# Daniel-Liu-c0deb0t/block-aligner

Hardware: AMD Instinct MI355X
Metric: GCUPS (DP cells/s) on 10 kbp DNA X-drop batch; bit-exact score+CIGAR vs AVX2 (higher is better)
Workload: dtype i16 (saturating lane scores) + i32 block offsets

## Files before the change

block_aligner_amd/csrc/ba_host.cpp:

```cpp
#include <hip/hip_runtime.h>

#include <algorithm>
#include <functional>
#include <cmath>
#include <cstdarg>
#include <cstdio>
#include <cstdlib>
#include <cstring>
#include <map>
#include <memory>
#include <string>
#include <type_traits>
#include <vector>
#include <atomic>
#include <chrono>
#include <thread>

#include "../../include/block_aligner_hip.h"
#include "aa_matrices.inc"
#include "ba_launch.h"

using ba::BatchParams;
using ba::BlockRec;

typedef const ba::KernelEntry* KernelTable[2][ba::N_KINDS][ba::N_CLASSES][ba::FAM_COUNT];
static KernelTable& kernel_table() { static KernelTable t = {}; return t; }
int ba::register_kernels(int kind, int pmax, bool special, const ba::KernelEntry* entries, int n) {
    int pc = 0;
    while ((1 << pc) < pmax) pc++;
    for (int k = 0; k < n; k++) kernel_table()[special][kind][pc][entries[k].family] = &entries[k];
    return n;
}
static const ba::KernelEntry* find_kernel(int family, int kind, int pc, int special) {
    if (family < 0 || family >= ba::FAM_COUNT || kind < 0 || kind >= ba::N_KINDS || pc < 0 || pc >= ba::N_CLASSES || special < 0 || special > 1) return nullptr;
    return kernel_table()[special][kind][pc][family];
}
constexpr int BA_PCLASS_BIG = 5;
static inline int special_of(uint32_t mode) { return (mode & (BA_LOCAL_START | BA_FREE_QUERY_START_GAPS | BA_FREE_QUERY_END_GAPS)) ? 1 : 0; }
constexpr int BA_KIND_PROFILE_ = ba::KIND_PROFILE;

#ifdef BA_DEV
#define dev_env(name) getenv(name)
#else
#define dev_env(name) ((const char*)nullptr)
#endif
#ifndef BA_BUILD_ID
#define BA_BUILD_ID "unknown"
#endif
extern "C" const char* ba_build_id(void) { return BA_BUILD_ID; }
extern "C" int ba_dev_build(void) {
#ifdef BA_DEV
    return 1;
#else
    return 0;
#endif
}

static thread_local std::string g_err;
static int fail(const char* fmt, ...) {
    char buf[512];
    va_list ap; va_start(ap, fmt); vsnprintf(buf, sizeof buf, fmt, ap); va_end(ap);
    g_err = buf;
    return 1;
}
[[noreturn]] static void die(const char* fmt, ...) {
    char buf[512];
    va_list ap; va_start(ap, fmt); vsnprintf(buf, sizeof buf, fmt, ap); va_end(ap);
    fprintf(stderr, "block_aligner_hip: %s\n", buf);
    abort();
}
#define HIP_TRY(expr) do { hipError_t e_ = (expr); if (e_ != hipSuccess) return fail("%s failed: %s", #expr, hipGetErrorString(e_)); } while (0)

static thread_local int g_device = -1;
static int ensure_device() {
    int n = 0;
    hipError_t e = hipGetDeviceCount(&n);
    if (e != hipSuccess || n <= 0) return fail("no usable HIP device (hipGetDeviceCount: %s); block_aligner_hip has no CPU fallback", hipGetErrorString(e));
    if (g_device < 0) g_device = 0;
    HIP_TRY(hipSetDevice(g_device));
    return 0;
}

struct AAMatrix { alignas(32) int8_t scores[27 * 32]; };
struct NucMatrix { alignas(32) int8_t scores[8 * 16]; };

static constexpr AAMatrix expand_tri(const signed char* tri) {
    AAMatrix m{};
    for (int k = 0; k < 27 * 32; k++) m.scores[k] = -128;
    int idx = 0;
    const char* letters = BA_AA_LETTERS;
    for (int a = 0; a < BA_AA_NLETTERS; a++)
        for (int b = 0; b <= a; b++) {
            const int ia = letters[a] - 'A', ib = letters[b] - 'A';
            m.scores[ia * 32 + ib] = tri[idx];
            m.scores[ib * 32 + ia] = tri[idx];
            idx++;
        }
    return m;
}
static constexpr NucMatrix nuc_simple(int8_t match, int8_t mismatch) {
    NucMatrix m{};
    for (int k = 0; k < 8 * 16; k++) m.scores[k] = -128;
    const char alpha[5] = {'A', 'T', 'C', 'G', 'N'};
    for (int i = 0; i < 5; i++)
        for (int j = 0; j < 5; j++) m.scores[(alpha[i] & 7) * 16 + (alpha[j] & 15)] = i == j ? match : mismatch;
    return m;
}
extern "C" {
extern const NucMatrix NW1 = nuc_simple(1, -1);
extern const AAMatrix BLOSUM45 = expand_tri(BA_TRI_BLOSUM45);
extern const AAMatrix BLOSUM50 = expand_tri(BA_TRI_BLOSUM50);
extern const AAMatrix BLOSUM62 = expand_tri(BA_TRI_BLOSUM62);
extern const AAMatrix BLOSUM80 = expand_tri(BA_TRI_BLOSUM80);
extern const AAMatrix BLOSUM90 = expand_tri(BA_TRI_BLOSUM90);
extern const AAMatrix PAM100 = expand_tri(BA_TRI_PAM100);
extern const AAMatrix PAM120 = expand_tri(BA_TRI_PAM120);
extern const AAMatrix PAM160 = expand_tri(BA_TRI_PAM160);
extern const AAMatrix PAM200 = expand_tri(BA_TRI_PAM200);
extern const AAMatrix PAM250 = expand_tri(BA_TRI_PAM250);
extern const ByteMatrix BYTES1 = {1, -1};
}

static inline uint8_t upper(uint8_t c) { return (c >= 'a' && c <= 'z') ? (uint8_t)(c - 32) : c; }
static inline int seq_kind(int kind) { return kind == BA_KIND_PROFILE_ ? BA_KIND_AA : kind; }
static inline uint8_t null_byte(int kind) { kind = seq_kind(kind); return kind == BA_KIND_AA ? 26 : (kind == BA_KIND_NUC ? 'Z' : 0); }
static inline bool convert_char(int kind, uint8_t c, uint8_t* out) {
    kind = seq_kind(kind);
    if (kind == BA_KIND_BYTES) { *out = c; return true; }
    c = upper(c);
    if (kind == BA_KIND_AA) { if (c < 'A' || c > 'A' + 26) return false; *out = (uint8_t)(c - 'A'); return true; }
    if (c < 'A' || c > 'Z') return false;
    *out = c;
    return true;
}

struct PaddedBytes {
    std::vector<uint8_t> s;
    size_t len;
    int kind;
};
struct Cigar {
    std::vector<OpLen> ops;
    size_t capacity;
};
struct AAProfile {
    std::vector<int8_t> pos_aa;
    std::vector<int16_t> gap_open_C, gap_close_C, gap_open_R;
    int8_t gap_extend;
    size_t max_len, curr_len, str_len;
};

struct DevBuf {
    void* p = nullptr;
    size_t bytes = 0;
    bool owned = true;
    void view(void* q, size_t n) { free_(); p = q; bytes = n; owned = false; }
    int alloc(size_t n) {
        free_();
        owned = true;
        if (n == 0) n = 4;
        hipError_t e = hipMalloc(&p, n);
        if (e != hipSuccess) { p = nullptr; return fail("hipMalloc(%zu bytes) failed: %s", n, hipGetErrorString(e)); }
        bytes = n;
        return 0;
    }
    void free_() { if (p && owned) (void)hipFree(p); p = nullptr; bytes = 0; }
    ~DevBuf() { free_(); }
    template <class T> T* as() const { return (T*)p; }
};

struct TextState {
    DevBuf len, off, pos, buf;
    uint64_t buf_cap = 0, run = 0;
    uint32_t what = ~0u;
    bool sized = false;
    hipEvent_t ev[2] = {};
    float ms = 0;
    ~TextState() { for (hipEvent_t e : ev) if (e) (void)hipEventDestroy(e); }
};

struct BaBatch {
    int device = 0;
    hipStream_t stream = nullptr, stream2 = nullptr;
    hipEvent_t ev0 = nullptr, ev1 = nullptr, ev_fork = nullptr, ev_join = nullptr, ev_l0 = nullptr, ev_m1 = nullptr;
    int kind = 0; uint32_t mode = 0;
    uint32_t n = 0, min_size = 0, max_size = 0, pclass = 0;
    int gap_open = 0, gap_extend = 0, x_drop = 0;
    uint32_t grid = 0, lds = 0, slots = 0;
    uint64_t trace_stride = 0, blocks_stride = 0, cig_total = 0, pool_bytes = 0;
    uint64_t trace_full = 0;
    bool adaptive = false;
    bool opt_class = false;
    bool bet_lost = false;
    uint64_t plan_fixed = 0, plan_maxlen2 = 0, plan_avg = 0;
    uint32_t retried = 0;
    uint64_t cap_n = 0, cap_pool = 0, cap_cig = 0, cap_maxlen2 = 0;
    DevBuf pool, q_off, q_len, r_off, r_len, matrix, score, qidx, ridx, cig_ops, cig_off, cig_len, cells, status, nblocks, pair_slot, trace_words, trace, blocks, ckpt, big, counter,
           tb_queue, tb_ctrl, slot_free, slot_info, prof, params_dev, donate;
    std::vector<uint32_t> h_order;
    uint32_t tb_stride = 0, n_fill_waves = 0, slots_per_wave = 1, tb_qsize = 1, tb_reserve = 0;
    std::vector<uint64_t> h_q_off, h_r_off;
    bool ran = false, in_flight = false;
    uint32_t work_chunk = 1;
    uint32_t mq_drain = 0;
    bool multi = false;
    uint32_t multi_b = 128;
    uint32_t geom = 0;
    uint32_t wpw = ba::WAVES_PER_WG;
    uint32_t walk_wave_n = 0;
    uint32_t sm_excl_n = 0;
    uint32_t sm_side_n = 0;
    bool small = false;
    bool quad = false;
    DevBuf contA, cont_n;
    DevBuf cq_queue, cq_ctrl;
    uint32_t quad_grid = 0, cq_grid = 0;
    bool pipe = false;
    DevBuf trace_off, blocks_off;
    uint64_t pipe_words = 0, pipe_recs = 0;
    DevBuf compact, compact_off, compact_total, dev_of;
    DevBuf stats, stats_pos;
    hipEvent_t ev_s0 = nullptr, ev_s1 = nullptr;
    float stats_ms = 0;
    DevBuf ex_rows, ex_work, ex_out, ex_counter;
    hipEvent_t ev_x0 = nullptr, ev_x1 = nullptr;
    float exact_ms = 0; uint64_t exact_cells = 0;
    DevBuf xt_trace, xt_rev, xt_rev_off, xt_nrun, xt_off, xt_runs;
    float xt_ms = 0; uint64_t xt_cells = 0;
    bool xt_valid = false; uint32_t xt_what = 0; int32_t xt_x_drop = 0; uint64_t xt_loads = 0;
    std::vector<uint32_t> xt_devpos; std::vector<BaExact> xt_out; std::vector<uint64_t> xt_h_off;
    int xt_form = 0;
    float xp_ms = 0; uint64_t xp_cells = 0;
    DevBuf xt_start; std::vector<uint32_t> xt_h_start;
    uint64_t loads = 0;
    TextState text;
    uint64_t runs_done = 0;
    uint64_t compact_cap = 0, compact_used_cap = 0; bool compacted = false; uint32_t* compact_host = nullptr;
    unsigned long long* h_total = nullptr;
    bool pad_negative = false;
    bool handle_mode = false;
    DevBuf hblk, rblk;
    BatchParams params() const {
        BatchParams bp{};
        bp.pool = pool.as<uint8_t>();
        bp.q_off = q_off.as<uint64_t>(); bp.q_len = q_len.as<uint32_t>();
        bp.r_off = r_off.as<uint64_t>(); bp.r_len = r_len.as<uint32_t>();
        bp.n = n; bp.gap_open = gap_open; bp.gap_extend = gap_extend;
        bp.min_size = min_size; bp.max_size = max_size; bp.x_drop = x_drop; bp.flags = mode | (dev_env("BA_NO_FAST") ? 0x100u : 0u) | ((dev_env("BA_SKIP_WALK") || dev_env("BA_NO_TRACEBACK")) ? 0x200u : 0u) | ((handle_mode || dev_env("BA_NO_SPEC")) ? 0x400u : 0u) | (dev_env("BA_NO_TB_WAVES") ? 0x800u : 0u) | (dev_env("BA_NO_REFILL") ? 0x1000u : 0u) | (dev_env("BA_NO_STEAL") ? 0x2000u : 0u) | ((pad_negative && !dev_env("BA_NO_END_CLIP")) ? (uint32_t)ba::F_PAD_NEG : 0u) | (((uint64_t)pool.bytes + 2ull * max_size + 8ull > 0xffffffffull || dev_env("BA_POOL64")) ? (uint32_t)ba::F_POOL64 : 0u);
        bp.matrix = matrix.as<int8_t>();
        bp.score = score.as<int32_t>(); bp.query_idx = qidx.as<uint32_t>(); bp.reference_idx = ridx.as<uint32_t>();
        bp.cig_ops = ((mode & BA_TRACE) && !handle_mode && !dev_env("BA_NO_TRACEBACK")) ? cig_ops.as<uint32_t>() : nullptr;
        bp.cig_off = cig_off.as<uint64_t>(); bp.cig_start = nullptr; bp.cig_len = cig_len.as<uint32_t>();
        bp.cells = cells.as<unsigned long long>(); bp.status = status.as<uint32_t>(); bp.nblocks_out = nblocks.as<uint32_t>(); bp.slot_out = pair_slot.as<uint32_t>(); bp.trace_words_out = trace_words.as<uint32_t>();
        bp.walk_wave_n = walk_wave_n;
        bp.trace_arena = trace.as<uint32_t>(); bp.trace_stride = trace_stride;
        bp.blocks = blocks.as<BlockRec>(); bp.blocks_stride = blocks_stride;
        bp.trace_off = pipe ? trace_off.as<uint64_t>() : nullptr; bp.blocks_off = pipe ? blocks_off.as<uint64_t>() : nullptr;
        bp.ckpt = ckpt.as<short>(); bp.big = big.as<short>();
        bp.tb_stride = tb_stride; bp.slots_per_wave = slots_per_wave; bp.n_slots = slots; bp.tb_reserve = tb_reserve;
        bp.tb_qmask = tb_qsize - 1;
        bp.tb_queue = tb_queue.as<uint32_t>(); bp.tb_ctrl = tb_ctrl.as<uint32_t>();
        bp.slot_free = slot_free.as<uint32_t>(); bp.slot_info = slot_info.as<ba::SlotInfo>();
        bp.work_counter = counter.as<uint32_t>();
        bp.work_chunk = work_chunk;
        bp.mq_drain = mq_drain;
        bp.mq_waves = grid * wpw;
        bp.mq_donate = (multi && (mode & BA_TRACE) && !special_of(mode) && donate.p && !dev_env("BA_NO_DONATE")) ? donate.as<uint32_t>() : nullptr;
        bp.sm_excl_n = small ? sm_excl_n : 0; bp.sm_excl_first = 0;
        bp.prof = prof.as<unsigned long long>();
        return bp;
    }
    ~BaBatch() {
        if (ev0) (void)hipEventDestroy(ev0);
        if (ev1) (void)hipEventDestroy(ev1);
        if (ev_fork) (void)hipEventDestroy(ev_fork);
        if (ev_join) (void)hipEventDestroy(ev_join);
        if (h_total) (void)hipHostFree(h_total);
        if (ev_l0) (void)hipEventDestroy(ev_l0);
        if (ev_m1) (void)hipEventDestroy(ev_m1);
        if (ev_s0) (void)hipEventDestroy(ev_s0);
        if (ev_s1) (void)hipEventDestroy(ev_s1);
        if (ev_x0) (void)hipEventDestroy(ev_x0);
        if (ev_x1) (void)hipEventDestroy(ev_x1);
        if (stream2) (void)hipStreamDestroy(stream2);
        if (stream) (void)hipStreamDestroy(stream);
    }
};

static int check_align_params(bool profile, Gaps g, size_t min_size, size_t max_size, int32_t x_drop, uint32_t mode, std::string* why, bool linear_ok = false) {
    if (profile) { if (!(g.extend < 0)) { *why = "Gap extend cost must be negative!"; return 1; } }
    else {
        if (!(g.open < 0 && g.extend < 0)) { *why = "Gap costs must be negative!"; return 1; }
        if (!(g.open < g.extend) && !(linear_ok && g.open == g.extend)) { *why = "Gap open must cost more than gap extend!"; return 1; }
    }
    if (!(min_size < 65535 && max_size < 65535)) { *why = "Block sizes must be smaller than 2^16 - 1!"; return 1; }
    if ((min_size & (min_size - 1)) || (max_size & (max_size - 1))) { *why = "Block sizes must be powers of two!"; return 1; }
    if ((mode & BA_X_DROP) && x_drop < 0) { *why = "X-drop threshold amount must be nonnegative!"; return 1; }
    if ((mode & BA_LOCAL_START) && (mode & BA_FREE_QUERY_START_GAPS)) { *why = "Cannot set both LOCAL_START and FREE_QUERY_START_GAPS!"; return 1; }
    if ((mode & BA_X_DROP) && (mode & BA_FREE_QUERY_END_GAPS)) { *why = "Cannot set both X_DROP and FREE_QUERY_END_GAPS!"; return 1; }
    return 0;
}

constexpr size_t BA_MAX_BLOCK = 32768;
static int pclass_of(size_t max_size) {
    if (max_size <= 128) return 0;
    if (max_size == 256) return 1;
    if (max_size == 512) return 2;
    if (max_size == 1024) return 3;
    if (max_size == 2048) return 4;
    if (max_size == 4096 || max_size == 8192 || max_size == 16384 || max_size == 32768) return BA_PCLASS_BIG;
    return -1;
}
static inline uint32_t lds_class_cells(int pc) { return pc == BA_PCLASS_BIG ? 128u : 128u << pc; }

static void profile_image(const AAProfile* pr, uint32_t P, uint8_t* dst) {
    int8_t* pos_aa = (int8_t*)dst;
    int16_t* aa_pos = (int16_t*)(dst + (size_t)P * 32);
    int16_t* goC = aa_pos + (size_t)P * 32; int16_t* clC = goC + P; int16_t* goR = clC + P;
    const size_t have = std::min<size_t>(P, pr->curr_len);
    memset(pos_aa, 0x80, (size_t)P * 32);
    memcpy(pos_aa, pr->pos_aa.data(), have * 32);
    for (size_t c = 0; c < 32; c++)
        for (size_t i = 0; i < P; i++) aa_pos[c * P + i] = (int16_t)pos_aa[i * 32 + c];
    for (size_t i = 0; i < P; i++) {
        goC[i] = i < have ? pr->gap_open_C[i] : (int16_t)-128;
        clC[i] = i < have ? pr->gap_close_C[i] : (int16_t)-128;
        goR[i] = i < have ? pr->gap_open_R[i] : (int16_t)-128;
    }
}
struct NoProfiles { const AAProfile* operator()(size_t) const { return nullptr; } };

constexpr size_t POOL_SLACK = 256;
struct ExtImages {
    const uint8_t* host_base = nullptr; const uint8_t* dev_base = nullptr;
    const uint8_t* flags = nullptr;
    const uint32_t* seed_of = nullptr;
    float* pack_ms = nullptr;
};
struct Packed {
    std::vector<uint64_t> qo, ro, cig_off;
    std::vector<uint32_t> ql, rl;
    std::vector<uint8_t> image;
    uint64_t total = 0, maxlen2 = 0, cig_total = 0;
    bool on_device = false;
    const uint8_t* raw = nullptr; uint64_t raw_bytes = 0; uint32_t pad = 0;
    std::vector<uint64_t> raw_qo, raw_ro;
    const ExtImages* ext = nullptr; std::vector<uint8_t> ext_flags;
    std::vector<uint32_t> order;
    size_t who(size_t s) const { return order.empty() ? s : order[s]; }
};
template <class GetSeq, class GetProfile, class Lap>
static int pack_pairs_in_order(int kind, Gaps gaps, size_t min_size, size_t max_size, uint32_t mode, size_t n, bool already_converted,
                               GetSeq get, GetProfile getp, Packed& P, Lap lap, const ExtImages* ext = nullptr) {
    const bool profile = kind == BA_KIND_PROFILE_;
    const size_t pad = max_size + 16;
    std::vector<uint64_t>& qo = P.qo; std::vector<uint64_t>& ro = P.ro;
    qo.resize(n); ro.resize(n);
    std::vector<uint32_t>& ql = P.ql; std::vector<uint32_t>& rl = P.rl;
    ql.resize(n); rl.resize(n);
    uint64_t total = 0, maxlen2 = 0, cig_total = 0;
    std::vector<uint64_t>& cig_off = P.cig_off;
    cig_off.resize(n + 1);
    const uint8_t* lo = nullptr; const uint8_t* hi = nullptr; uint64_t sum_len = 0;
    auto span = [&](const uint8_t* ptr, size_t len) {
        if (!lo || ptr < lo) lo = ptr;
        if (!hi || ptr + len > hi) hi = ptr + len;
        sum_len += len;
    };
    for (size_t p = 0; p < n; p++) {
        const uint8_t* ptr; size_t len;
        get(p, 0, &ptr, &len);
        if (len > 0x3fffffffu) { fail("sequence too long"); return 1; }
        span(ptr, len);
        ql[p] = (uint32_t)len; qo[p] = total; total += (1 + len + pad + 3) & ~(size_t)3;
        if ((mode & BA_FREE_QUERY_END_GAPS) && !(min_size > len)) {
            fail("pair %zu: Min block size must be larger than the query length for FREE_QUERY_END_GAPS!", P.who(p)); return 1;
        }
        if (profile) {
            const AAProfile* pr = getp(p);
            if (!pr) { fail("pair %zu: null profile", P.who(p)); return 1; }
            if (pr->gap_extend != gaps.extend) { fail("pair %zu: profile gap_extend %d differs from the batch's %d", P.who(p), pr->gap_extend, gaps.extend); return 1; }
            len = pr->str_len;
            if (len > 0x3fffffffu) { fail("profile too long"); return 1; }
            rl[p] = (uint32_t)len; ro[p] = total; total += ba::profile_image_bytes((uint32_t)len, (uint32_t)max_size);
        } else {
            get(p, 1, &ptr, &len);
            if (len > 0x3fffffffu) { fail("sequence too long"); return 1; }
            span(ptr, len);
            rl[p] = (uint32_t)len; ro[p] = total; total += (1 + len + pad + 3) & ~(size_t)3;
        }
        maxlen2 = std::max<uint64_t>(maxlen2, (uint64_t)ql[p] + rl[p] + 2);
        cig_off[p] = cig_total;
        cig_total += (uint64_t)ql[p] + rl[p] + 1;
    }
    cig_off[n] = cig_total;
    total += POOL_SLACK;
    lap("offsets");
    P.total = total; P.maxlen2 = maxlen2; P.cig_total = cig_total; P.pad = (uint32_t)pad;
    if (ext) {
        P.on_device = true; P.ext = ext; P.raw = ext->host_base;
        P.raw_qo.resize(n); P.raw_ro.resize(n); P.ext_flags.resize(2 * n);
        for (size_t p = 0; p < n; p++) {
            const uint8_t* ptr; size_t len;
            get(p, 0, &ptr, &len); P.raw_qo[p] = (uint64_t)(ptr - ext->host_base);
            get(p, 1, &ptr, &len); P.raw_ro[p] = (uint64_t)(ptr - ext->host_base);
            P.ext_flags[2 * p] = ext->flags[2 * P.who(p)]; P.ext_flags[2 * p + 1] = ext->flags[2 * P.who(p) + 1];
        }
        lap("extension image offsets");
        return 0;
    }
    if (!profile && !already_converted && n >= 256 && n < (1u << 30) && (uint64_t)(hi - lo) <= 2 * sum_len + 4096 && !dev_env("BA_HOST_PACK")) {
        P.on_device = true; P.raw = lo; P.raw_bytes = (uint64_t)(hi - lo);
        P.raw_qo.resize(n); P.raw_ro.resize(n);
        for (size_t p = 0; p < n; p++) {
            const uint8_t* ptr; size_t len;
            get(p, 0, &ptr, &len); P.raw_qo[p] = (uint64_t)(ptr - lo);
            get(p, 1, &ptr, &len); P.raw_ro[p] = (uint64_t)(ptr - lo);
        }
        lap("raw offsets");
        return 0;
    }
    std::vector<uint8_t>& image = P.image;
    image.assign(total, null_byte(kind));
    lap("image allocation + padding");
    {
        unsigned nthreads = std::thread::hardware_concurrency();
        if (nthreads > 16) nthreads = 16;
        if (nthreads < 1 || n < 4096) nthreads = 1;
        std::vector<size_t> bad(nthreads, (size_t)-1);
        std::vector<uint8_t> bad_byte(nthreads, 0);
        auto work = [&](unsigned t) {
            for (size_t p = (size_t)n * t / nthreads; p < (size_t)n * (t + 1) / nthreads; p++) {
                if (profile) profile_image(getp(p), ba::profile_positions(rl[p], (uint32_t)max_size), image.data() + ro[p]);
                for (int w = 0; w < (profile ? 1 : 2); w++) {
                    const uint8_t* ptr; size_t len;
                    get(p, w, &ptr, &len);
                    uint8_t* dst = image.data() + (w ? ro[p] : qo[p]) + 1;
                    if (already_converted) memcpy(dst, ptr, len);
                    else for (size_t k = 0; k < len; k++) {
                        if (!convert_char(kind, ptr[k], dst + k)) { if (bad[t] == (size_t)-1) { bad[t] = p; bad_byte[t] = ptr[k]; } break; }
                    }
                }
            }
        };
        std::vector<std::thread> th;
        for (unsigned t = 1; t < nthreads; t++) th.emplace_back(work, t);
        work(0);
        for (auto& x : th) x.join();
        for (unsigned t = 0; t < nthreads; t++)
            if (bad[t] != (size_t)-1) { fail("pair %zu: byte 0x%02x is outside the matrix alphabet", P.who(bad[t]), bad_byte[t]); return 1; }
    }
    lap("image fill");
    P.total = total; P.maxlen2 = maxlen2; P.cig_total = cig_total;
    return 0;
}

template <class GetSeq, class GetProfile, class Lap>
static int pack_pairs(int kind, Gaps gaps, size_t min_size, size_t max_size, uint32_t mode, size_t n, bool already_converted,
                      GetSeq get, GetProfile getp, Packed& P, Lap lap, const ExtImages* ext = nullptr) {
    std::vector<uint64_t> cost(n);
    for (size_t p = 0; p < n; p++) {
        const uint8_t* ptr; size_t len;
        get(p, 0, &ptr, &len); cost[p] = len;
        if (kind == BA_KIND_PROFILE_) { const AAProfile* pr = getp(p); cost[p] += pr ? pr->str_len : 0; }
        else { get(p, 1, &ptr, &len); cost[p] += len; }
    }
    P.order.resize(n);
    for (size_t p = 0; p < n; p++) P.order[p] = (uint32_t)p;
    std::stable_sort(P.order.begin(), P.order.end(), [&](uint32_t a, uint32_t c) { return cost[a] > cost[c]; });
    bool identity = true;
    for (size_t p = 0; p < n && identity; p++) identity = P.order[p] == p;
    if (identity || dev_env("BA_CALLER_ORDER")) P.order.clear();
    lap("longest-first order");
    const std::vector<uint32_t>& order = P.order;
    if (order.empty()) return pack_pairs_in_order(kind, gaps, min_size, max_size, mode, n, already_converted, get, getp, P, lap, ext);
    return pack_pairs_in_order(kind, gaps, min_size, max_size, mode, n, already_converted,
                               [&](size_t s, int w, const uint8_t** ptr, size_t* len) { get(order[s], w, ptr, len); },
                               [&](size_t s) { return getp(order[s]); }, P, lap, ext);
}

static void pipe_regions(const BaBatch* b, const uint32_t* ql, const uint32_t* rl, size_t n, uint64_t pct, std::vector<uint64_t>& toff,
                         std::vector<uint64_t>& boff) {
    toff.resize(n + 1); boff.resize(n + 1);
    const uint64_t mx = b->max_size, mn = b->min_size;
    const uint64_t zm = (b->mode & BA_LOCAL_START) ? 2 : 1;
    uint64_t t = b->small ? 512ull * 32 * 64 * 16 + 64 : 0, r = 0;
    t = (t + 15) & ~15ull;
    for (size_t p = 0; p < n; p++) {
        const uint64_t len2 = (uint64_t)ql[p] + rl[p] + 2;
        const uint64_t full = (mx / 16) * (len2 + 2 * mx) * 2 * zm + 64;
        const uint64_t want = (len2 * mn / 8 + mx * mx / 8 + 16 * mx) * zm * pct / 100 + 4096;
        toff[p] = t; t += (std::min(want, full) + 15) & ~15ull;
        boff[p] = r; r += len2 / 4 + 64;
    }
    toff[n] = t; boff[n] = r;
}
static thread_local uint64_t g_mem_cap = ~0ull;
static void mem_info(size_t* free_b, size_t* total_b) {
    *free_b = 0; *total_b = 0;
    (void)hipMemGetInfo(free_b, total_b);
    if ((uint64_t)*free_b > g_mem_cap) *free_b = (size_t)g_mem_cap;
}
static int pipe_cut(BaBatch* b, const uint32_t* ql, const uint32_t* rl, size_t n, uint64_t fixed_bytes, std::vector<uint64_t>& toff, std::vector<uint64_t>& boff) {
    size_t free_b = 0, total_b = 0;
    mem_info(&free_b, &total_b);
    uint64_t forced = 0;
    if (const char* env = dev_env("BA_TRACE_MARGIN_PCT")) { int v = atoi(env); if (v > 0) forced = (uint64_t)v; }
    const bool local = b->mode & BA_LOCAL_START;
    for (uint64_t pct : {local ? 300ull : 175ull, local ? 175ull : 140ull, 110ull}) {
        if (forced) pct = forced;
        pipe_regions(b, ql, rl, n, pct, toff, boff);
        if (b->pipe_words) { if (toff[n] <= b->pipe_words && boff[n] <= b->pipe_recs) return 0; }
        else if (toff[n] * 4 + boff[n] * sizeof(BlockRec) + fixed_bytes + (1ull << 30) <= (uint64_t)free_b * 85 / 100) return 0;
    }
    return 1;
}

static ba::KernelFamily family_of(const BaBatch* b) {
    if (b->pclass == BA_PCLASS_BIG) return ba::FAM_TILED;
    if (b->multi) return b->geom == 2 ? ba::FAM_MULTI_G2 : (b->geom ? ba::FAM_MULTI_G3 : (b->multi_b == 512 ? ba::FAM_MULTI_512 : (b->multi_b == 256 ? ba::FAM_MULTI_256 : ba::FAM_MULTI)));
    return b->small ? ba::FAM_SMALL : ba::FAM_PAIR;
}
static const ba::KernelEntry* kernel_of(const BaBatch* b, bool quad = false) {
    const int family = quad ? ba::FAM_QUAD : family_of(b), pc = quad ? 0 : (int)b->pclass, special = quad ? 0 : special_of(b->mode);
    const ba::KernelEntry* k = find_kernel(family, b->kind, pc, special);
    if (!k) fail("no kernel of family %d for kind %d, block class %d, %s modes", family, b->kind, pc, special ? "special" : "plain");
    return k;
}
static uint32_t kernel_lds_bytes(const BaBatch* b) {
    const uint32_t cells = lds_class_cells((int)b->pclass);
    switch (family_of(b)) {
    case ba::FAM_PAIR: case ba::FAM_TILED:
        return ba::lds_wg_bytes_h(b->kind, cells) + ((b->mode & BA_TRACE) ? (special_of(b->mode) ? ba::TB_LDS_BYTES_LOC : ba::TB_LDS_BYTES) : 0u);
    case ba::FAM_SMALL: return ba::sm_wg_bytes_h(b->kind, cells);
    default: return ba::mq_wg_bytes_h(b->kind, cells, b->wpw);
    }
}
static size_t kernel_wave_arena_bytes(const BaBatch* b) {
    switch (family_of(b)) {
    case ba::FAM_PAIR: return 0;
    case ba::FAM_TILED: return ba::big_wave_shorts(b->max_size) * sizeof(short);
    case ba::FAM_SMALL: return ba::SM_WAVE_BYTES;
    default: return ba::MQ_WAVE_BYTES;
    }
}
static const void* kernel_fn(const BaBatch* b, const ba::KernelEntry* k, bool trace, int form) { return k->fn[form][trace][(b->mode & BA_X_DROP) != 0]; }
static hipError_t kernel_lds_opt_in(const void* fn, unsigned lds) {
    return lds > 64 * 1024 ? hipFuncSetAttribute(fn, hipFuncAttributeMaxDynamicSharedMemorySize, (int)lds) : hipSuccess;
}
static hipError_t kernel_launch(const BaBatch* b, const ba::KernelEntry* k, bool trace, unsigned grid, unsigned lds, hipStream_t s, const BatchParams* bp) {
    const void* fn = kernel_fn(b, k, trace, (k->fn[1][0][0] && !(bp->flags & ba::F_LOCAL)) ? 1 : 0);
    if (hipError_t e = kernel_lds_opt_in(fn, lds)) return e;
    void* args[] = {(void*)bp};
    return hipLaunchKernel(fn, dim3(grid), dim3(k->wpw * 64), args, lds, s);
}
static hipError_t kernel_occupancy(const BaBatch* b, const ba::KernelEntry* k, bool trace, unsigned lds, int* blocks_per_cu) {
    *blocks_per_cu = 0;
    for (int form = 0; form < 2 && k->fn[form][0][0]; form++) {
        const void* fn = kernel_fn(b, k, trace, form);
        int v = 0;
        if (hipError_t e = kernel_lds_opt_in(fn, lds)) return e;
        if (hipError_t e = hipOccupancyMaxActiveBlocksPerMultiprocessor(&v, fn, (int)k->wpw * 64, lds)) return e;
        *blocks_per_cu = form ? std::min(*blocks_per_cu, v) : v;
    }
    return hipSuccess;
}
static int quad_grid(const BaBatch* b, uint32_t* grid) {
    const ba::KernelEntry* k = kernel_of(b, true);
    if (!k) return 1;
    int per_cu = 0, dev = 0;
    hipDeviceProp_t prop;
    if (kernel_occupancy(b, k, (b->mode & BA_TRACE) != 0, k->lds, &per_cu) != hipSuccess || hipGetDevice(&dev) != hipSuccess || hipGetDeviceProperties(&prop, dev) != hipSuccess)
        return fail("occupancy query failed for the small-block kernel");
    per_cu = std::max(1, std::min(per_cu, 32 / (int)k->wpw));
    *grid = (uint32_t)(prop.multiProcessorCount * per_cu);
    return *grid ? 0 : fail("occupancy query failed for the small-block kernel");
}

static int batch_plan(BaBatch* b, size_t n, uint64_t fixed_bytes, uint64_t maxlen2, bool full_trace, uint64_t avg_len2 = ~0ull) {
    const int kind = b->kind; const uint32_t mode = b->mode; const int pc = (int)b->pclass; const size_t max_size = b->max_size;
    const bool trace = mode & BA_TRACE;
    hipDeviceProp_t prop;
    if (hipGetDeviceProperties(&prop, b->device) != hipSuccess) { fail("hipGetDeviceProperties failed"); return 1; }
    const ba::KernelEntry* k = kernel_of(b);
    if (!k) return 1;
    b->lds = kernel_lds_bytes(b);
    if (b->lds > 160 * 1024) { fail("block size %zu needs %u bytes of LDS per workgroup", max_size, b->lds); return 1; }
    int per_cu = 0;
    if (kernel_occupancy(b, k, trace, b->lds, &per_cu) != hipSuccess || per_cu <= 0) {
        fail("occupancy query failed for kind %d class %d (lds %u)", kind, pc, b->lds); return 1;
    }
    if (per_cu * b->wpw > 32) per_cu = 32 / b->wpw;
    if (b->geom && per_cu > (int)b->geom) per_cu = (int)b->geom;
    if (const char* env = dev_env("BA_WGS_PER_CU")) { int v = atoi(env); if (v > 0) per_cu = v; }
    uint64_t grid = (uint64_t)prop.multiProcessorCount * per_cu;
    const uint64_t per_wg = (uint64_t)b->wpw * (b->small ? ba::SM_SLOTS : ((b->multi && b->geom && !trace) ? 512u / b->multi_b : 1u));
    const uint64_t need = (n + per_wg - 1) / per_wg;
    if (grid > need) grid = need;
    if (const char* env = dev_env("BA_GRID")) { int v = atoi(env); if (v > 0 && (uint64_t)v < grid) grid = (uint64_t)v; }
    const uint64_t zm = (mode & BA_LOCAL_START) ? 2 : 1;
    b->trace_full = trace ? (uint64_t)(max_size / 16) * (maxlen2 + 2 * max_size) * 2 * zm + 64 : 0;
    b->trace_stride = b->trace_full;
    b->adaptive = false;
    if (trace && !full_trace && !dev_env("BA_FULL_TRACE_SLOTS") && (n >= 4096 || (maxlen2 >= 20000 && n >= 256) || g_mem_cap != ~0ull || dev_env("BA_ADAPTIVE_TRACE"))) {
        const uint64_t est = (maxlen2 * b->min_size / 8 + (uint64_t)max_size * max_size / 8 + 16ull * max_size) * zm;
        uint64_t pct = ((mode & BA_LOCAL_START) && maxlen2 <= 4096) ? 500 : 175;
        if (b->multi && !(mode & BA_LOCAL_START)) pct = 125;
        if (const char* env = dev_env("BA_TRACE_MARGIN_PCT")) { int v = atoi(env); if (v > 0) pct = (uint64_t)v; }
        const uint64_t want = est * pct / 100 + 4096;
        if (want < b->trace_full) { b->trace_stride = (want + 15) & ~15ull; b->adaptive = true; }
    }
    b->blocks_stride = trace ? maxlen2 : 0;
    if (b->trace_stride >= (1ull << 30)) { fail("trace stack of %llu words per pair exceeds the 2^30 limit", (unsigned long long)b->trace_stride); return 1; }
    if (trace) {
        size_t free_b = 0, total_b = 0;
        mem_info(&free_b, &total_b);
        const uint64_t per_slot = b->trace_stride * 4 + b->blocks_stride * sizeof(BlockRec);
        const uint64_t fixed = fixed_bytes + (1ull << 30);
        const uint64_t budget = free_b * 9 / 10 > fixed ? free_b * 9 / 10 - fixed : 0;
        const uint64_t max_waves = per_slot ? budget / per_slot : ~0ull;
        if (max_waves < b->wpw) { fail("device memory: one workgroup's trace slots need %llu MB, %llu MB are free", (unsigned long long)(per_slot * b->wpw >> 20), (unsigned long long)(budget >> 20)); return 1; }
        if (grid * b->wpw > max_waves) grid = max_waves / b->wpw;
    }
    if (b->small) grid = std::min<uint64_t>(grid, 512ull * 32 / b->wpw);
    b->grid = (uint32_t)grid;
    b->cq_grid = 0;
    if (b->quad) {
        b->cq_grid = (uint32_t)std::min<uint64_t>(grid, (uint64_t)prop.multiProcessorCount);
        if (const char* env = dev_env("BA_CQ_GRID")) { int v = atoi(env); if (v > 0) b->cq_grid = (uint32_t)std::min<uint64_t>(grid, (uint64_t)v); }
    }
    b->tb_stride = 0; b->slots_per_wave = 1;
    b->n_fill_waves = b->grid * b->wpw;
    const bool short_pairs = kind != BA_KIND_PROFILE_ && avg_len2 <= 1024 && !dev_env("BA_FORCE_TB");
    {
        const uint64_t waves = grid * b->wpw;
        const uint64_t by_len = avg_len2 != ~0ull ? 16384 / (avg_len2 + 1) : 1, by_n = waves ? n / (waves * 8) : 1;
        b->work_chunk = (uint32_t)std::max<uint64_t>(1, std::min<uint64_t>(8, std::min(by_len, by_n)));
        if (b->small) b->work_chunk = 4;
        if (b->small && n >= 2 * waves * ba::SM_SLOTS) b->work_chunk = 8;
        if (const char* env = dev_env("BA_WORK_CHUNK")) { int v = atoi(env); if (v > 0) b->work_chunk = (uint32_t)v; }
    }
    uint64_t few_x = lds_class_cells(pc) >= 512 ? 2u : 1u;
    if (const char* env = dev_env("BA_FEW_PAIRS_X")) { int v = atoi(env); if (v >= 0) few_x = (uint64_t)v; }
    const bool few_pairs = !special_of(mode) && n <= few_x * (uint64_t)grid * b->wpw && !dev_env("BA_FORCE_TB");
    if (trace && (b->grid >= 32 || (dev_env("BA_FORCE_TB") && b->grid >= 2)) && !short_pairs && !few_pairs && !b->pipe && !dev_env("BA_INLINE_TRACEBACK")) {
        uint32_t stride = b->grid >= 32 ? (b->min_size >= 128 ? 4 : 3) : 2;
        if (b->multi && b->grid >= 32) stride = 2;
        if (b->multi && b->grid >= 32 && !special_of(mode)) stride = 3;
        if (b->multi && b->geom && b->grid >= 32) stride = 6;
        if (const char* env = dev_env("BA_TB_STRIDE")) { int v = atoi(env); if (v > 0) stride = (uint32_t)v; }
        b->tb_stride = stride;
        b->n_fill_waves = b->grid * b->wpw - (b->grid + stride - 1) / stride;
        size_t free_b = 0, total_b = 0;
        mem_info(&free_b, &total_b);
        const uint64_t per_slot = b->trace_stride * 4 + b->blocks_stride * sizeof(BlockRec);
        const uint64_t fixed = fixed_bytes + (1ull << 30);
        uint32_t spw = 4;
        const uint32_t mslots = b->multi ? 512u / b->multi_b : 0u;
        if (b->multi) spw = mslots + 5;
        if (const char* env = dev_env("BA_SLOTS_PER_WAVE")) { int v = atoi(env); if (v > 0) spw = (uint32_t)v; }
        while (spw > 1 && fixed + per_slot * spw * b->n_fill_waves > free_b * 9 / 10) spw--;
        if (b->multi && spw < mslots + 2) return fail("device memory: the multi-pair kernel needs two trace slots per wave beside its pairs'");
        b->slots_per_wave = spw;
        b->tb_reserve = b->n_fill_waves / 2;
        if (b->multi && (n >= 5ull * b->n_fill_waves || !special_of(mode)) && spw >= mslots + 2) b->tb_reserve = b->n_fill_waves;
        if (spw < 3) b->tb_reserve = b->n_fill_waves / 4;
        if (const char* env = dev_env("BA_TB_RESERVE")) b->tb_reserve = (uint32_t)std::max(0, atoi(env));
        if (b->multi) b->tb_reserve = std::min<uint32_t>(b->tb_reserve, b->n_fill_waves * (spw > mslots ? spw - mslots : 1) - 1);
    }
    b->mq_drain = b->multi ? ((dev_env("BA_NO_DONATE") || !trace || special_of(mode)) ? b->n_fill_waves : b->n_fill_waves / 4) : 0;
    if (const char* env = dev_env("BA_MQ_DRAIN")) b->mq_drain = (uint32_t)std::max(0, atoi(env));
    if (b->multi && b->slots_per_wave < 512u / b->multi_b) b->slots_per_wave = 512u / b->multi_b;
    b->slots = b->n_fill_waves * b->slots_per_wave;
    if (b->pipe) b->slots = (uint32_t)n;
    {
        const uint64_t lanes = b->tb_stride ? (uint64_t)((b->grid + b->tb_stride - 1) / b->tb_stride) * 64 + b->n_fill_waves : 0;
        uint64_t need_q = std::max<uint64_t>(lanes, b->slots);
        uint32_t qs = 1;
        while (qs < need_q) qs <<= 1;
        b->tb_qsize = qs;
    }

    return 0;
}
static int batch_alloc_scratch(BaBatch* b) {
#define BA_ALLOC(buf, bytes) if (b->buf.alloc(bytes)) return 1
    BA_ALLOC(trace, b->pipe ? b->pipe_words * 4 : b->trace_stride * 4 * b->slots);
    BA_ALLOC(blocks, b->pipe ? b->pipe_recs * sizeof(BlockRec) : b->blocks_stride * sizeof(BlockRec) * b->slots);
    BA_ALLOC(ckpt, (size_t)(b->grid + b->cq_grid) * b->wpw * 8 * b->max_size * sizeof(short));
    BA_ALLOC(big, (size_t)b->grid * b->wpw * kernel_wave_arena_bytes(b));
    BA_ALLOC(tb_queue, (size_t)b->tb_qsize * 4); BA_ALLOC(tb_ctrl, 256); BA_ALLOC(prof, 2048); BA_ALLOC(params_dev, sizeof(BatchParams));
    BA_ALLOC(slot_free, (size_t)b->slots * 4); BA_ALLOC(slot_info, (size_t)b->slots * sizeof(ba::SlotInfo)); BA_ALLOC(counter, 128);
    if (b->multi) BA_ALLOC(donate, ((size_t)b->grid * b->wpw + 64) * 4);
#undef BA_ALLOC
    return 0;
}

static int upload_images(BaBatch* b, const Packed& P, size_t n) {
    if (!P.on_device) { HIP_TRY(hipMemcpy(b->pool.p, P.image.data(), P.total, hipMemcpyHostToDevice)); return 0; }
    if (P.ext) {
        DevBuf raw_q, raw_r, flags, err;
        if (raw_q.alloc(n * 8) || raw_r.alloc(n * 8) || flags.alloc(2 * n) || err.alloc(8)) return 1;
        HIP_TRY(hipMemcpy(raw_q.p, P.raw_qo.data(), n * 8, hipMemcpyHostToDevice));
        HIP_TRY(hipMemcpy(raw_r.p, P.raw_ro.data(), n * 8, hipMemcpyHostToDevice));
        HIP_TRY(hipMemcpy(flags.p, P.ext_flags.data(), 2 * n, hipMemcpyHostToDevice));
        HIP_TRY(hipMemset(err.p, 0xff, 8));
        HIP_TRY(hipMemset((uint8_t*)b->pool.p + P.total - POOL_SLACK, null_byte(b->kind), POOL_SLACK));
        HIP_TRY(hipEventRecord(b->ev0, b->stream));
        HIP_TRY(ba_launch_pack_images(b->stream, seq_kind(b->kind), P.ext->dev_base, raw_q.as<uint64_t>(), raw_r.as<uint64_t>(), flags.as<uint8_t>(),
                                      b->q_off.as<uint64_t>(), b->q_len.as<uint32_t>(), b->r_off.as<uint64_t>(), b->r_len.as<uint32_t>(),
                                      b->pool.as<uint8_t>(), P.pad, (uint32_t)n, err.as<unsigned long long>()));
        HIP_TRY(hipEventRecord(b->ev1, b->stream));
        HIP_TRY(hipStreamSynchronize(b->stream));
        if (P.ext->pack_ms) HIP_TRY(hipEventElapsedTime(P.ext->pack_ms, b->ev0, b->ev1));
        unsigned long long e = 0;
        HIP_TRY(hipMemcpy(&e, err.p, 8, hipMemcpyDeviceToHost));
        if (e != ~0ull) return fail("seed %u: byte 0x%02x is outside the matrix alphabet", P.ext->seed_of[P.who((size_t)(e >> 8))], (unsigned)(e & 0xff));
        return 0;
    }
    DevBuf raw, raw_q, raw_r, err;
    if (raw.alloc(P.raw_bytes) || raw_q.alloc(n * 8) || raw_r.alloc(n * 8) || err.alloc(8)) return 1;
    HIP_TRY(hipMemcpy(raw.p, P.raw, P.raw_bytes, hipMemcpyHostToDevice));
    HIP_TRY(hipMemcpy(raw_q.p, P.raw_qo.data(), n * 8, hipMemcpyHostToDevice));
    HIP_TRY(hipMemcpy(raw_r.p, P.raw_ro.data(), n * 8, hipMemcpyHostToDevice));
    HIP_TRY(hipMemset(err.p, 0xff, 8));
    HIP_TRY(hipMemset((uint8_t*)b->pool.p + P.total - POOL_SLACK, null_byte(b->kind), POOL_SLACK));
    HIP_TRY(ba_launch_pack_sequences(b->stream, seq_kind(b->kind), raw.as<uint8_t>(), raw_q.as<uint64_t>(), raw_r.as<uint64_t>(),
                                     b->q_off.as<uint64_t>(), b->q_len.as<uint32_t>(), b->r_off.as<uint64_t>(), b->r_len.as<uint32_t>(),
                                     b->pool.as<uint8_t>(), P.pad, (uint32_t)n, err.as<unsigned long long>()));
    HIP_TRY(hipStreamSynchronize(b->stream));
    unsigned long long e = 0;
    HIP_TRY(hipMemcpy(&e, err.p, 8, hipMemcpyDeviceToHost));
    if (e != ~0ull) return fail("pair %zu: byte 0x%02x is outside the matrix alphabet", P.who((size_t)(e >> 8)), (unsigned)(e & 0xff));
    return 0;
}

static bool pad_negative(int kind, const void* matrix) {
    const int8_t* m = (const int8_t*)matrix;
    if (!m) return false;
    if (kind == BA_KIND_NUC) {
        const int row = 'Z' & 7, col = 'Z' & 15;
        for (int a = 0; a < 16; a++) if (m[row * 16 + a] >= 0) return false;
        for (int c = 0; c < 8; c++) if (m[c * 16 + col] >= 0) return false;
        return true;
    }
    if (kind == BA_KIND_AA) {
        for (int a = 0; a < 27; a++) if (m[26 * 32 + a] >= 0 || m[a * 32 + 26] >= 0) return false;
        return true;
    }
    return false;
}
static int upload_dev_of(BaBatch* b);
static void plan_walks(BaBatch* b, const std::vector<uint32_t>& ql, const std::vector<uint32_t>& rl);
static void plan_exclusive(BaBatch* b, const std::vector<uint32_t>& ql, const std::vector<uint32_t>& rl);
template <class GetSeq, class GetProfile = NoProfiles>
static BaBatch* batch_build(int kind, const void* matrix, Gaps gaps, SizeRange size, int32_t x_drop, uint32_t mode, size_t n,
                            bool already_converted, GetSeq get, GetProfile getp = GetProfile(), const ExtImages* ext = nullptr) {
    if (ensure_device()) return nullptr;
    const bool verbose = dev_env("BA_SETUP_TIMING") != nullptr;
    auto t_last = std::chrono::steady_clock::now();
    auto lap = [&](const char* what) {
        if (!verbose) return;
        const auto now = std::chrono::steady_clock::now();
        fprintf(stderr, "block_aligner_hip setup: %-28s %8.1f ms\n", what, std::chrono::duration<double, std::milli>(now - t_last).count());
        t_last = now;
    };
    if (kind < 0 || kind > 3) { fail("unknown matrix kind %d", kind); return nullptr; }
    const bool profile = kind == BA_KIND_PROFILE_;
    const size_t min_size = size.min < 16 ? 16 : size.min, max_size = size.max < 16 ? 16 : size.max;
    std::string why;
    if (check_align_params(profile, gaps, min_size, max_size, x_drop, mode, &why, !ext)) { fail("%s", why.c_str()); return nullptr; }
    if (min_size > max_size) { fail("min block size exceeds max block size"); return nullptr; }
    if (profile && (mode & BA_CIGAR_EQ)) { fail("=/X CIGARs need two sequences; a profile alignment has none to compare"); return nullptr; }
    if (kind == BA_KIND_BYTES && (mode & BA_X_DROP)) {  }
    int pc = pclass_of(max_size);
    if (pc < 0) { fail("max block size %zu not supported by the HIP backend (16..%zu)", max_size, (size_t)BA_MAX_BLOCK); return nullptr; }
    if (n == 0 || n > 0x7fffffffu) { fail("batch must hold between 1 and 2^31-1 pairs"); return nullptr; }
    bool opt_class = false;
    if (pc == BA_PCLASS_BIG && min_size >= 128 && min_size <= 1024 && !dev_env("BA_NO_OPT_CLASS")) { pc = 4; opt_class = true; }

    std::unique_ptr<BaBatch> b(new BaBatch);
    b->device = g_device; b->kind = kind; b->mode = mode; b->n = (uint32_t)n;
    b->min_size = (uint32_t)min_size; b->max_size = (uint32_t)max_size; b->pclass = (uint32_t)pc; b->opt_class = opt_class;
    b->gap_open = gaps.open; b->gap_extend = gaps.extend; b->x_drop = x_drop;

    Packed P;
    if (pack_pairs(kind, gaps, min_size, max_size, mode, n, already_converted, get, getp, P, lap, ext)) return nullptr;
    std::vector<uint64_t>& qo = P.qo; std::vector<uint64_t>& ro = P.ro; std::vector<uint32_t>& ql = P.ql; std::vector<uint32_t>& rl = P.rl;
    std::vector<uint64_t>& cig_off = P.cig_off;
    const uint64_t total = P.total, maxlen2 = P.maxlen2, cig_total = P.cig_total;
    b->h_q_off = qo; b->h_r_off = ro; b->h_order = P.order;
    plan_walks(b.get(), ql, rl);
    b->cap_n = n; b->cap_pool = total; b->cap_cig = cig_total; b->cap_maxlen2 = maxlen2;
    b->pool_bytes = total;

    if (hipStreamCreateWithFlags(&b->stream, hipStreamNonBlocking) != hipSuccess) { fail("hipStreamCreate failed"); return nullptr; }
    if (hipEventCreate(&b->ev0) != hipSuccess || hipEventCreate(&b->ev1) != hipSuccess) { fail("hipEventCreate failed"); return nullptr; }

    const bool trace = mode & BA_TRACE;
    const size_t mat_bytes = kind == BA_KIND_AA ? 27 * 32 : (kind == BA_KIND_NUC ? 8 * 16 : (profile ? 0 : 2));
    uint64_t sum_len2 = 0;
    for (size_t p = 0; p < n; p++) sum_len2 += (uint64_t)ql[p] + rl[p];
    const size_t quad_from = kind == BA_KIND_AA ? 65536u : 8192u;
    const bool trace_mode = mode & BA_TRACE;
    b->quad = !special_of(mode) && pc != BA_PCLASS_BIG && min_size == 32 && !dev_env("BA_NO_QUAD") && (dev_env("BA_FORCE_QUAD") || n >= quad_from);
    size_t small_from = kind == BA_KIND_AA ? (trace_mode ? 98304u : 32768u) : (trace_mode ? 57344u : 49152u);
    if (profile) small_from = 10000u;
    const bool small_mode = !special_of(mode) || (!profile && !(mode & BA_FREE_QUERY_END_GAPS));
    if (mode & BA_LOCAL_START) small_from = trace_mode ? 196608u : 262144u;
    if ((mode & BA_FREE_QUERY_START_GAPS) && !dev_env("BA_FORCE_SMALL")) small_from = ~(size_t)0;
    b->small = small_mode && pc <= 3 && min_size == ba::SM_B_HOST && !dev_env("BA_NO_SMALL") && (dev_env("BA_FORCE_SMALL") || (n >= small_from && !dev_env("BA_FORCE_QUAD")));
    if (b->small) b->quad = false;
    std::vector<uint64_t> toff, boff;
    if (trace && (!special_of(mode) || b->small) && pc != BA_PCLASS_BIG && (b->quad || b->small || (profile && n >= 4096) || dev_env("BA_FORCE_PIPE"))) {
        const uint64_t fixed = total + cig_total * 4 + (uint64_t)n * (64 + sizeof(ba::PairCont) + 40);
        if (!dev_env("BA_NO_PIPE") && !pipe_cut(b.get(), ql.data(), rl.data(), n, fixed, toff, boff)) {
            b->pipe = true; b->pipe_words = toff[n] + toff[n] / 8; b->pipe_recs = boff[n] + boff[n] / 8;
        }
    }
    if (trace && !b->pipe) b->quad = b->small = false;
    const uint64_t avg_len2 = n ? sum_len2 / n : 0;
    bool multi_fits = avg_len2 >= 3000 ? n >= 10000 : (!trace_mode && n >= 49152);
    b->multi_b = 128;
    bool wide = false;
    if (min_size == 256 && kind == BA_KIND_NUC && !special_of(mode) && max_size >= 512 && pc >= 2 && pc <= 4) {
        wide = true; b->multi_b = 256;
        multi_fits = avg_len2 >= 6000 && n >= 256;
    }
    b->geom = 0; b->wpw = ba::WAVES_PER_WG;
    const bool geom_ok = !wide && kind == BA_KIND_NUC && !special_of(mode) && (pc == 2 || pc == 3) && min_size == ba::MQ_B_HOST;
    if (geom_ok && avg_len2 >= 3000) {
        int cus = 0;
        if (hipDeviceGetAttribute(&cus, hipDeviceAttributeMultiprocessorCount, b->device) != hipSuccess || cus <= 0) cus = 256;
        const uint64_t s2 = 32ull * (uint64_t)cus, s3 = 48ull * (uint64_t)cus;
        if (trace_mode) {
            b->geom = n <= s2 * 115 / 100 ? 2u : (n <= s3 * 136 / 100 ? 3u : 0u);
            multi_fits = n >= s2 * 65 / 100;
        } else {
            b->geom = n <= s2 * 113 / 100 ? 2u : (n <= s3 * 124 / 100 ? 3u : 0u);
            multi_fits = n >= s2 * 92 / 100;
        }
    }
    if (const char* env = dev_env("BA_MQ_GEOM")) { const int v = atoi(env); b->geom = (geom_ok && (v == 2 || v == 3)) ? (uint32_t)v : 0u; }
    if (min_size == 512 && kind == BA_KIND_NUC && !special_of(mode) && max_size >= 1024 && pc >= 3 && pc <= 4) {
        wide = true; b->multi_b = 512;
        multi_fits = avg_len2 >= 8000 && n >= 256;
    }
    b->multi = !profile && small_mode && pc != BA_PCLASS_BIG && (min_size == ba::MQ_B_HOST || wide) && !dev_env("BA_NO_MULTI") && (dev_env("BA_FORCE_MULTI") || multi_fits);
    if (!b->multi) { b->multi_b = 128; b->geom = 0; }
// ... 2285 lines not shown
```

block_aligner_amd/csrc/ba_kernels.hip:

```cpp
#include "ba_driver.hpp"
#include "ba_launch.h"

#ifndef BA_KIND
#error "define BA_KIND"
#endif
#ifndef BA_PMAX
#error "define BA_PMAX"
#endif

#ifndef BA_SPECIAL
#define BA_SPECIAL 0
#endif

#if !BA_BIG && (BA_KIND != 3 || (!BA_SPECIAL && BA_PMAX <= 8))
#include "ba_multi.hpp"
#endif
#if !BA_BIG && BA_PMAX <= 8 && (BA_KIND != 3 || !BA_SPECIAL)
#include "ba_small.hpp"
#endif
#if !BA_BIG && BA_PMAX == 1 && !BA_SPECIAL
#include "ba_quad.hpp"
#endif

#define K_ALIGN(T, X) ba::k_align<BA_PMAX, BA_KIND, T, X, (BA_SPECIAL != 0)>
#define K_MULTI(T, X) ba::k_multi<BA_PMAX, BA_KIND, T, X>
#define K_MULTI_256(T, X) ba::k_multi<BA_PMAX, BA_KIND, T, X, 0, 256>
#define K_MULTI_512(T, X) ba::k_multi<BA_PMAX, BA_KIND, T, X, 0, 512>
#define K_MULTI_G2(T, X) ba::k_multi<BA_PMAX, BA_KIND, T, X, 0, 128, ba::MQ_GEOM_WPW, 2>
#define K_MULTI_G3(T, X) ba::k_multi<BA_PMAX, BA_KIND, T, X, 0, 128, ba::MQ_GEOM_WPW, 3>
#define K_MULTI_S1(T, X) ba::k_multi<BA_PMAX, BA_KIND, T, X, 1>
#define K_MULTI_S2(T, X) ba::k_multi<BA_PMAX, BA_KIND, T, X, 2>
#define K_SMALL(T, X) ba::k_small<BA_PMAX, BA_KIND, T, X>
#define K_SMALL_S1(T, X) ba::k_small<BA_PMAX, BA_KIND, T, X, 1>
#define K_SMALL_S2(T, X) ba::k_small<BA_PMAX, BA_KIND, T, X, 2>
#define K_QUAD(T, X) ba::k_quad<BA_KIND, T, X>
#define BA_TX(K) {{(const void*)K(false, false), (const void*)K(false, true)}, {(const void*)K(true, false), (const void*)K(true, true)}}
#define BA_ENTRY(FAM, WPW, K) {FAM, WPW, 0u, {BA_TX(K), {}}}
#define BA_ENTRY_SPM(FAM, WPW, K1, K2) {FAM, WPW, 0u, {BA_TX(K1), BA_TX(K2)}}

static const ba::KernelEntry g_entries[] = {
    BA_ENTRY(BA_BIG ? ba::FAM_TILED : ba::FAM_PAIR, ba::WAVES_PER_WG, K_ALIGN),
#if BA_KIND != 3 && !BA_SPECIAL && !BA_BIG
    BA_ENTRY(ba::FAM_MULTI, ba::WAVES_PER_WG, K_MULTI),
#if BA_KIND == 1 && BA_PMAX >= 4
    BA_ENTRY(ba::FAM_MULTI_256, ba::WAVES_PER_WG, K_MULTI_256),
#endif
#if BA_KIND == 1 && BA_PMAX >= 8
    BA_ENTRY(ba::FAM_MULTI_512, ba::WAVES_PER_WG, K_MULTI_512),
#endif
#if BA_KIND == 1 && (BA_PMAX == 4 || BA_PMAX == 8)
    BA_ENTRY(ba::FAM_MULTI_G3, ba::MQ_GEOM_WPW, K_MULTI_G3),
    BA_ENTRY(ba::FAM_MULTI_G2, ba::MQ_GEOM_WPW, K_MULTI_G2),
#endif
#endif
#if !BA_SPECIAL && !BA_BIG && BA_PMAX <= 8
    BA_ENTRY(ba::FAM_SMALL, ba::WAVES_PER_WG, K_SMALL),
#endif
#if BA_SPECIAL && !BA_BIG && BA_KIND != 3
    BA_ENTRY_SPM(ba::FAM_MULTI, ba::WAVES_PER_WG, K_MULTI_S1, K_MULTI_S2),
#endif
#if BA_SPECIAL && !BA_BIG && BA_PMAX <= 8 && BA_KIND != 3
    BA_ENTRY_SPM(ba::FAM_SMALL, ba::WAVES_PER_WG, K_SMALL_S1, K_SMALL_S2),
#endif
#if BA_PMAX == 1 && !BA_SPECIAL && !BA_BIG
    {ba::FAM_QUAD, ba::WAVES_PER_WG, ba::lds_table_bytes_h(BA_KIND) + ba::WAVES_PER_WG * 4 * ba::QUAD_SLOT_BYTES, {BA_TX(K_QUAD), {}}},
#endif
};
[[maybe_unused]] static const int g_registered = ba::register_kernels(BA_KIND, BA_PMAX, BA_SPECIAL != 0, g_entries, (int)(sizeof g_entries / sizeof g_entries[0]));

#if BA_KIND == 0 && BA_PMAX == 1 && !BA_SPECIAL && !BA_BIG
__global__ void __launch_bounds__(64) k_traceback(const ba::BatchParams bp) {
    using namespace ba;
    __shared__ uint32_t words[4096];
    uint32_t st = 0, n = 0;
    if (bp.flags & (F_LOCAL | F_FQS)) {
        if (lane_id() == 0)
            n = traceback(bp.blocks + (uint64_t)bp.tb_slot * bp.blocks_stride, bp.tb_nblocks, bp.trace_arena + (uint64_t)bp.tb_slot * bp.trace_stride, bp.tb_i,
                          bp.tb_j, bp.pool + bp.q_off[0], bp.pool + bp.r_off[0], bp.flags, bp.cig_ops, bp.cig_off[0], bp.cig_off[1], &st);
    } else
        n = walk_wave<false>(bp.blocks + (uint64_t)bp.tb_slot * bp.blocks_stride, bp.tb_nblocks, bp.trace_arena + (uint64_t)bp.tb_slot * bp.trace_stride, bp.tb_i,
                             bp.tb_j, bp.pool + bp.q_off[0], bp.pool + bp.r_off[0], (bp.flags & F_CIGAR_EQ) != 0, bp.cig_ops, bp.cig_off[0], bp.cig_off[1], &st,
                             words, 4096u);
    if (lane_id() == 0) { bp.cig_len[0] = n; bp.status[0] = st; }
}

__global__ void __launch_bounds__(64) k_lane_kat(int form, const short* __restrict__ x, short* __restrict__ out, int gap_extend) {
    using namespace ba;
    const int lane = lane_id();
    if (form >= 5) {
        const short* xi = x + (size_t)blockIdx.x * 512 + lane * 8;
        int r[4];
#pragma unroll
        for (int k = 0; k < 4; k++) r[k] = pk((int)xi[k], (int)xi[k + 4]);
        const int ge2 = splat(gap_extend);
        const int l = lane & (form == 5 ? 15 : (form == 6 ? 31 : 63));
        const MultiConsts mc = make_multi_consts(l, gap_extend);
        const int r3 = scan_halves(r, ge2, mc);
        const int cs = form == 5 ? multi_carry<16>(r3, mc, l) : (form == 6 ? multi_carry<32>(r3, mc, l) : multi_carry<64>(r3, mc, l));
        apply_halves(r, r3, cs, ge2, mc);
        short* oi = out + (size_t)blockIdx.x * 512 + lane * 8;
#pragma unroll
        for (int k = 0; k < 4; k++) { oi[k] = as_s(r[k]).x; oi[k + 4] = as_s(r[k]).y; }
        return;
    }
    if (form <= 1) {
        const short* xi = x + (size_t)blockIdx.x * 512 + lane * 8;
        int xr[4], r[4];
#pragma unroll
        for (int k = 0; k < 4; k++) xr[k] = pk((int)xi[2 * k], (int)xi[2 * k + 1]);
        const int ge2 = splat(gap_extend);
#pragma unroll
        for (int k = 0; k < 4; k++) r[k] = scan8_inreg(xr[k], ge2);
        int G[4], cs;
        if (form == 0) {
            const MultiConsts mc = make_multi_consts(lane & 15, gap_extend);
#pragma unroll
            for (int k = 0; k < 4; k++) G[k] = pk(max(-32768, (2 * k + 1) * gap_extend), max(-32768, (2 * k + 2) * gap_extend));
            scan8_chain(r, G[0]);
            cs = multi_carry(r[3], mc);
        } else {
            const SmallConsts mc = make_small_consts(lane & 3, gap_extend);
#pragma unroll
            for (int k = 0; k < 4; k++) G[k] = mc.G[k];
            scan8_chain(r, G[0]);
            cs = small_carry(r[3], mc, lane & 3);
        }
        short* oi = out + (size_t)blockIdx.x * 512 + lane * 8;
#pragma unroll
        for (int k = 0; k < 4; k++) { const int v = scan8_apply(r[k], cs, G[k], k == 3); oi[2 * k] = as_s(v).x; oi[2 * k + 1] = as_s(v).y; }
    } else {
        const int nl = form == 2 ? 64 : (form == 3 ? 32 : 16);
        const size_t base = (size_t)blockIdx.x * (size_t)(2 * nl);
        const int xv = lane < nl ? pk((int)x[base + 2 * lane], (int)x[base + 2 * lane + 1]) : 0;
        const FillConsts fc = make_fill_consts(lane, 0, gap_extend);
        const int v = form == 2 ? fast_scan<64>(xv, fc) : (form == 3 ? fast_scan<32>(xv, fc) : fast_scan<16>(xv, fc));
        if (lane < nl) { out[base + 2 * lane] = as_s(v).x; out[base + 2 * lane + 1] = as_s(v).y; }
    }
}
extern "C" hipError_t ba_launch_lane_kat(hipStream_t s, int form, const short* x, short* out, int gap_extend, unsigned waves) {
    k_lane_kat<<<dim3(waves), dim3(64), 0, s>>>(form, x, out, gap_extend);
    return hipGetLastError();
}

constexpr int WALK_WAVES = 4;
__global__ void __launch_bounds__(WALK_WAVES * 64) k_walk(const ba::BatchParams bp) {
    extern __shared__ __attribute__((aligned(16))) unsigned char walk_lds[];
    ba::traceback_all(bp, (uint32_t)ba::F_CIGAR_EQ, walk_lds + ((uint32_t)threadIdx.x >> 6) * ba::TB_LDS_BYTES);
}

__global__ void __launch_bounds__(WALK_WAVES * 64) k_walk_l2(const ba::BatchParams bp) {
    extern __shared__ __attribute__((aligned(16))) unsigned char walk_lds[];
    ba::traceback_all<true>(bp, (uint32_t)ba::F_CIGAR_EQ, walk_lds + ((uint32_t)threadIdx.x >> 6) * ba::TB_LDS_BYTES_L2);
}

__global__ void __launch_bounds__(WALK_WAVES * 64) k_walk_loc(const ba::BatchParams bp) {
    extern __shared__ __attribute__((aligned(16))) unsigned char walk_lds[];
    ba::traceback_all<true, true>(bp, (uint32_t)ba::F_CIGAR_EQ, walk_lds + ((uint32_t)threadIdx.x >> 6) * ba::TB_LDS_BYTES_LOC);
}

__global__ void __launch_bounds__(256) k_compact_cigars(const uint32_t* __restrict__ ops, const uint64_t* __restrict__ cig_off,
                                                        const uint32_t* __restrict__ cig_len, const uint64_t* __restrict__ out_off,
                                                        uint32_t* __restrict__ out, uint32_t n) {
    for (uint32_t p = blockIdx.x; p < n; p += gridDim.x) {
        const uint32_t len = cig_len[p];
        const uint64_t src = cig_off[p + 1] - len, dst = out_off[p];
        for (uint32_t k = threadIdx.x; k < len; k += blockDim.x) out[dst + k] = ops[src + k];
    }
}
__global__ void __launch_bounds__(1024) k_cigar_offsets(const uint32_t* __restrict__ cig_len, const uint32_t* __restrict__ dev_of, uint64_t* __restrict__ out_off,
                                                        unsigned long long* __restrict__ total, uint32_t n) {
    __shared__ unsigned long long part[1024];
    const uint32_t t = threadIdx.x, per = (n + 1023u) / 1024u;
    const uint32_t lo = min(t * per, n), hi = min(lo + per, n);
    unsigned long long sum = 0;
    for (uint32_t p = lo; p < hi; p++) sum += cig_len[dev_of ? dev_of[p] : p];
    part[t] = sum;
    __syncthreads();
    for (uint32_t d = 1; d < 1024; d <<= 1) {
        const unsigned long long v = t >= d ? part[t - d] : 0ull;
        __syncthreads();
        part[t] += v;
        __syncthreads();
    }
    unsigned long long at = part[t] - sum;
    for (uint32_t p = lo; p < hi; p++) { const uint32_t s = dev_of ? dev_of[p] : p; out_off[s] = at; at += cig_len[s]; }
    if (t == 1023) *total = part[1023];
}
__global__ void __launch_bounds__(256) k_compact_cigars_checked(const uint32_t* __restrict__ ops, const uint64_t* __restrict__ cig_off,
                                                                const uint32_t* __restrict__ cig_len, const uint64_t* __restrict__ out_off,
                                                                uint32_t* __restrict__ out, uint32_t n, const unsigned long long* __restrict__ total, unsigned long long capacity) {
    if (*total > capacity) return;
    for (uint32_t p = blockIdx.x; p < n; p += gridDim.x) {
        const uint32_t len = cig_len[p];
        const uint64_t src = cig_off[p + 1] - len, dst = out_off[p];
        for (uint32_t k = threadIdx.x; k < len; k += blockDim.x) out[dst + k] = ops[src + k];
    }
}
extern "C" hipError_t ba_launch_cigar_offsets_and_compact(hipStream_t s, const uint32_t* ops, const uint64_t* cig_off, const uint32_t* cig_len, const uint32_t* dev_of,
                                                          uint64_t* out_off, uint32_t* out, unsigned long long* total, unsigned long long capacity, uint32_t n) {
    k_cigar_offsets<<<dim3(1), dim3(1024), 0, s>>>(cig_len, dev_of, out_off, total, n);
    const unsigned grid = n < 4096 ? (n ? n : 1) : 4096;
    k_compact_cigars_checked<<<dim3(grid), dim3(256), 0, s>>>(ops, cig_off, cig_len, out_off, out, n, total, capacity);
    return hipGetLastError();
}
extern "C" hipError_t ba_launch_compact_cigars(hipStream_t s, const uint32_t* ops, const uint64_t* cig_off, const uint32_t* cig_len,
                                               const uint64_t* out_off, uint32_t* out, uint32_t n) {
    const unsigned grid = n < 4096 ? (n ? n : 1) : 4096;
    k_compact_cigars<<<dim3(grid), dim3(256), 0, s>>>(ops, cig_off, cig_len, out_off, out, n);
    return hipGetLastError();
}
__global__ void __launch_bounds__(256) k_pack_sequences(int kind, const uint8_t* __restrict__ raw, const uint64_t* __restrict__ raw_q,
                                                        const uint64_t* __restrict__ raw_r, const uint64_t* __restrict__ q_off,
                                                        const uint32_t* __restrict__ q_len, const uint64_t* __restrict__ r_off,
                                                        const uint32_t* __restrict__ r_len, uint8_t* __restrict__ image, uint32_t pad,
                                                        unsigned long long* err) {
    const uint32_t p = blockIdx.x >> 1;
    const bool ref = blockIdx.x & 1;
    const uint8_t* src = raw + (ref ? raw_r[p] : raw_q[p]);
    const uint32_t len = ref ? r_len[p] : q_len[p];
    uint32_t* dst = (uint32_t*)(image + (ref ? r_off[p] : q_off[p]));
    const uint32_t null_b = kind == ba::KIND_AA ? 26u : (kind == ba::KIND_NUC ? (uint32_t)'Z' : 0u);
    const uint32_t words = ((1u + len + pad + 3u) & ~3u) / 4u;
    for (uint32_t k = threadIdx.x; k < words; k += blockDim.x) {
        uint32_t wd = 0;
#pragma unroll
        for (uint32_t b = 0; b < 4; b++) {
            const uint32_t pos = 4 * k + b;
            uint32_t c = null_b;
            if (pos >= 1 && pos <= len) {
                c = src[pos - 1];
                if (kind != ba::KIND_BYTES) {
                    if (c >= 'a' && c <= 'z') c -= 32;
                    const bool ok = kind == ba::KIND_AA ? (c >= 'A' && c <= 'A' + 26) : (c >= 'A' && c <= 'Z');
                    if (!ok) { atomicMin(err, ((unsigned long long)p << 8) | src[pos - 1]); c = null_b; }
                    else if (kind == ba::KIND_AA) c -= 'A';
                }
            }
            wd |= c << (8 * b);
        }
        dst[k] = wd;
    }
}
extern "C" hipError_t ba_launch_pack_sequences(hipStream_t s, int kind, const uint8_t* raw, const uint64_t* raw_q, const uint64_t* raw_r,
                                               const uint64_t* q_off, const uint32_t* q_len, const uint64_t* r_off, const uint32_t* r_len,
                                               uint8_t* image, uint32_t pad, uint32_t n, unsigned long long* err) {
    k_pack_sequences<<<dim3(2 * n), dim3(256), 0, s>>>(kind, raw, raw_q, raw_r, q_off, q_len, r_off, r_len, image, pad, err);
    return hipGetLastError();
}
__global__ void __launch_bounds__(256) k_merge_retry(const uint32_t* __restrict__ idx, const ba::BatchParams sub, const ba::BatchParams dst,
                                                     const uint32_t* __restrict__ sub_trace_words, uint32_t* __restrict__ dst_trace_words) {
    const uint32_t k = blockIdx.x, p = idx[k];
    const uint32_t len = sub.cig_len[k];
    if (threadIdx.x == 0) {
        dst.score[p] = sub.score[k]; dst.query_idx[p] = sub.query_idx[k]; dst.reference_idx[p] = sub.reference_idx[k];
        dst.cig_len[p] = len; dst.status[p] = sub.status[k]; dst.cells[p] = sub.cells[k];
        dst_trace_words[p] = sub_trace_words[k];
    }
    if (!sub.cig_ops || !dst.cig_ops) return;
    const uint64_t src = sub.cig_off[k + 1] - len, to = dst.cig_off[p + 1] - len;
    for (uint32_t t = threadIdx.x; t < len; t += blockDim.x) dst.cig_ops[to + t] = sub.cig_ops[src + t];
}
extern "C" hipError_t ba_launch_merge_retry(hipStream_t s, const uint32_t* idx, uint32_t k, const ba::BatchParams* sub, const ba::BatchParams* dst,
                                            const uint32_t* sub_tw, uint32_t* dst_tw) {
    k_merge_retry<<<dim3(k), dim3(256), 0, s>>>(idx, *sub, *dst, sub_tw, dst_tw);
    return hipGetLastError();
}
extern "C" hipError_t ba_launch_walk(hipStream_t s, const ba::BatchParams* bp, uint32_t grid) {
    k_walk<<<dim3(grid), dim3(WALK_WAVES * 64), WALK_WAVES * ba::TB_LDS_BYTES, s>>>(*bp);
    return hipGetLastError();
}
extern "C" hipError_t ba_launch_walk_l2(hipStream_t s, const ba::BatchParams* bp, uint32_t grid) {
    k_walk_l2<<<dim3(grid), dim3(WALK_WAVES * 64), WALK_WAVES * ba::TB_LDS_BYTES_L2, s>>>(*bp);
    return hipGetLastError();
}
extern "C" hipError_t ba_launch_walk_loc(hipStream_t s, const ba::BatchParams* bp, uint32_t grid) {
    k_walk_loc<<<dim3(grid), dim3(WALK_WAVES * 64), WALK_WAVES * ba::TB_LDS_BYTES_LOC, s>>>(*bp);
    return hipGetLastError();
}
extern "C" hipError_t ba_launch_traceback(hipStream_t s, const ba::BatchParams* bp) {
    k_traceback<<<dim3(1), dim3(64), 0, s>>>(*bp);
    return hipGetLastError();
}
#endif
```

block_aligner_amd/csrc/ba_launch.h:

```cpp
#pragma once
#include <hip/hip_runtime_api.h>

#include "ba_exact.h"
#include "ba_extend.h"
#include "ba_params.h"
#include "ba_stats.h"
#include "ba_text.h"

namespace ba {

enum KernelFamily {
    FAM_PAIR,
    FAM_TILED,
    FAM_MULTI,
    FAM_MULTI_256,
    FAM_MULTI_512,
    FAM_MULTI_G2,
    FAM_MULTI_G3,
    FAM_SMALL,
    FAM_QUAD,
    FAM_COUNT
};
constexpr int N_KINDS = 4, N_CLASSES = 6;

struct KernelEntry {
    KernelFamily family;
    unsigned wpw;
    unsigned lds;
    const void* fn[2][2][2];
};

int register_kernels(int kind, int pmax, bool special, const KernelEntry* entries, int n);

}

extern "C" {
hipError_t ba_launch_traceback(hipStream_t s, const ba::BatchParams* bp);
hipError_t ba_launch_lane_kat(hipStream_t s, int form, const short* x, short* out, int gap_extend, unsigned waves);
hipError_t ba_launch_walk(hipStream_t s, const ba::BatchParams* bp, uint32_t grid);
hipError_t ba_launch_walk_l2(hipStream_t s, const ba::BatchParams* bp, uint32_t grid);
hipError_t ba_launch_walk_loc(hipStream_t s, const ba::BatchParams* bp, uint32_t grid);
hipError_t ba_launch_merge_retry(hipStream_t s, const uint32_t* idx, uint32_t k, const ba::BatchParams* sub, const ba::BatchParams* dst,
                                 const uint32_t* sub_tw, uint32_t* dst_tw);
hipError_t ba_launch_compact_cigars(hipStream_t s, const uint32_t* ops, const uint64_t* cig_off, const uint32_t* cig_len,
                                    const uint64_t* out_off, uint32_t* out, uint32_t n);
hipError_t ba_launch_cigar_offsets_and_compact(hipStream_t s, const uint32_t* ops, const uint64_t* cig_off, const uint32_t* cig_len, const uint32_t* dev_of,
                                               uint64_t* out_off, uint32_t* out, unsigned long long* total, unsigned long long capacity, uint32_t n);
hipError_t ba_launch_pack_sequences(hipStream_t s, int kind, const uint8_t* raw, const uint64_t* raw_q, const uint64_t* raw_r,
                                    const uint64_t* q_off, const uint32_t* q_len, const uint64_t* r_off, const uint32_t* r_len,
                                    uint8_t* image, uint32_t pad, uint32_t n, unsigned long long* err);
hipError_t ba_launch_pack_images(hipStream_t s, int kind, const uint8_t* raw, const uint64_t* raw_q, const uint64_t* raw_r, const uint8_t* flags,
                                 const uint64_t* q_off, const uint32_t* q_len, const uint64_t* r_off, const uint32_t* r_len,
                                 uint8_t* image, uint32_t pad, uint32_t n, unsigned long long* err);
hipError_t ba_launch_extend_results(hipStream_t s, const ba::ExtendParams* ep);
hipError_t ba_launch_extend_gather(hipStream_t s, const ba::ExtendParams* ep);
hipError_t ba_launch_stats(hipStream_t s, const ba::StatsParams* sp);
hipError_t ba_launch_stats_extend(hipStream_t s, const ba::ExtendParams* ep, const ba::AlignStats* side, ba::AlignStats* out);
hipError_t ba_launch_exact(hipStream_t s, const ba::ExactParams* xp, uint32_t wgs);
hipError_t ba_launch_exact_trace(hipStream_t s, const ba::ExactParams* xp, uint32_t waves);
hipError_t ba_launch_exact_runs(hipStream_t s, const uint32_t* rev, const uint64_t* rev_off, const uint32_t* nrun, const uint64_t* off, uint32_t* runs,
                                uint32_t m);
hipError_t ba_launch_exact_seed(hipStream_t s, const ba::ExtendParams* ep, const uint32_t* which, uint32_t m, int32_t* out);
hipError_t ba_launch_exact_modes(hipStream_t s, const ba::ExactModeParams* mp, uint32_t wgs);
hipError_t ba_launch_exact_modes_trace(hipStream_t s, const ba::ExactModeParams* mp, uint32_t* start_cell, uint32_t waves);
hipError_t ba_launch_exact_join(hipStream_t s, const ba::ExactJoinParams* jp);
hipError_t ba_launch_text_len(hipStream_t s, const ba::TextParams* tp);
hipError_t ba_launch_text_write(hipStream_t s, const ba::TextParams* tp);
hipError_t ba_launch_offsets(hipStream_t s, const uint32_t* len, uint64_t* offsets, uint32_t n);
}
```

block_aligner_amd/csrc/ba_multi.hpp:

```cpp
#pragma once
#include "ba_quad.hpp"

namespace ba {
#ifndef MQ_SOLO_PRIO
#define MQ_SOLO_PRIO 2
#endif

template <int N>
__device__ __forceinline__ int row_bcast(int v) { return __builtin_amdgcn_update_dpp(v, v, 0x150 + N, 0xf, 0xf, false); }
__device__ __forceinline__ int row_shl1_keep(int last, int src) { return __builtin_amdgcn_update_dpp(last, src, 0x101, 0xf, 0xf, false); }
__device__ __forceinline__ int splat_hi(int x) { const s16x2 t = as_s(x); return as_i(s16x2{t.y, t.y}); }
__device__ __forceinline__ int splat_lo(int x) { const s16x2 t = as_s(x); return as_i(s16x2{t.x, t.x}); }

__device__ __forceinline__ int sel_mask(unsigned long long m, int a, int b) {
    int r;
    asm("v_cndmask_b32_e64 %0, %1, %2, %3" : "=v"(r) : "v"(b), "v"(a), "s"(m));
    return r;
}

template <int SL> __device__ __forceinline__ int slot_first(int v) {
    if constexpr (SL == 16) return row_bcast<0>(v);
    else if constexpr (SL == 64) return __builtin_amdgcn_readfirstlane(v);
    else return __builtin_amdgcn_ds_bpermute((lane_id() & 32) << 2, v);
}
template <int SL> __device__ __forceinline__ int slot_last(int v) {
    if constexpr (SL == 16) return row_bcast<15>(v);
    else if constexpr (SL == 64) return __builtin_amdgcn_readlane(v, 63);
    else return __builtin_amdgcn_ds_bpermute(((lane_id() & 32) + 31) << 2, v);
}
template <int SL> __device__ __forceinline__ int slot_shr1_z(int v, int l) {
    if constexpr (SL == 16) return row_shr1_z(v);
    else if constexpr (SL == 64) return wave_shr1_z(v);
    else { const int t = wave_shr1_z(v); return l == 0 ? 0 : t; }
}
template <int SL> __device__ __forceinline__ int slot_shl1_keep(int last, int src, int l) {
    if constexpr (SL == 16) return row_shl1_keep(last, src);
    else { const int t = __builtin_amdgcn_update_dpp(last, src, 0x130, 0xf, 0xf, false); return l == SL - 1 ? last : t; }
}

__device__ __forceinline__ void cells_split(int (&v)[4]) {
    const int a = v[0], b = v[1], c = v[2], d = v[3];
    v[0] = __builtin_amdgcn_perm(c, a, 0x05040100); v[1] = __builtin_amdgcn_perm(c, a, 0x07060302);
    v[2] = __builtin_amdgcn_perm(d, b, 0x05040100); v[3] = __builtin_amdgcn_perm(d, b, 0x07060302);
}
__device__ __forceinline__ void cells_join(int (&v)[4]) {
    const int a = v[0], b = v[1], c = v[2], d = v[3];
    v[0] = __builtin_amdgcn_perm(b, a, 0x05040100); v[1] = __builtin_amdgcn_perm(d, c, 0x05040100);
    v[2] = __builtin_amdgcn_perm(b, a, 0x07060302); v[3] = __builtin_amdgcn_perm(d, c, 0x07060302);
}
__device__ __forceinline__ int4 cells_split(int4 q) { int v[4] = {q.x, q.y, q.z, q.w}; cells_split(v); return int4{v[0], v[1], v[2], v[3]}; }
__device__ __forceinline__ int4 cells_join(int4 q) { int v[4] = {q.x, q.y, q.z, q.w}; cells_join(v); return int4{v[0], v[1], v[2], v[3]}; }
__device__ __forceinline__ int adds_lo(int a, int k) {
    int t;
    asm("v_pk_add_i16 %0, %1, %2 op_sel_hi:[0,1] clamp" : "=v"(t) : "v"(a), "s"(k));
    return t;
}
__device__ __forceinline__ int max_hi_lo(int a, int b) {
    asm("v_max_i16_sdwa %0, %0, %1 dst_sel:WORD_1 dst_unused:UNUSED_PRESERVE src0_sel:WORD_1 src1_sel:WORD_0" : "+v"(a) : "v"(b));
    return a;
}

struct MultiConsts {
    int g2, g3;
    int K4, G48;
    int laneKG, lanem1KG;
    int w0;
};

__device__ __forceinline__ MultiConsts make_multi_consts(int l, int gx) {
    MultiConsts mc;
    mc.laneKG = l * 8 * gx; mc.lanem1KG = l ? (l - 1) * 8 * gx : -32768;
    mc.g2 = splat(max(-32768, 2 * gx)); mc.g3 = splat(max(-32768, 3 * gx));
    mc.K4 = pk(0, max(-32768, 4 * gx)); mc.G48 = pk(max(-32768, 4 * gx), max(-32768, 8 * gx));
    mc.w0 = pk(0, l == 0 ? 0 : ((l & 1) ? max(-32768, 8 * l * gx) : 4 * gx));
    return mc;
}
template <int SL = 16>
__device__ __forceinline__ int multi_carry(int r3, const MultiConsts& mc, int l = 0) {
    if constexpr (SL == 16) {
        const int pm = wave_prefix_max16((int)as_s(r3).y - mc.laneKG);
        return vmax(scan8_splat_lo(add_row_shr1(pm, mc.lanem1KG)), mc.w0);
    } else {
        const int pm = SL == 64 ? wave_prefix_max((int)as_s(r3).y - mc.laneKG) : wave_prefix_max32((int)as_s(r3).y - mc.laneKG);
        const int cin = add_shr1(pm, mc.lanem1KG);
        return vmax(scan8_splat_lo(l == 0 ? -32768 : cin), mc.w0);
    }
}

__device__ __forceinline__ int scan_halves(int (&r)[4], int ge2, const MultiConsts& mc) {
#pragma unroll
    for (int k = 1; k < 4; k++) r[k] = vmax(r[k], adds(r[k - 1], ge2));
    return vmax(r[3], adds_lo(r[3], mc.K4));
}
__device__ __forceinline__ void apply_halves(int (&r)[4], int r3, int cs, int ge2, const MultiConsts& mc) {
    const int t = max_hi_lo(adds_lo(cs, mc.K4), r[3]);
    r[0] = vmax(r[0], adds(t, ge2)); r[1] = vmax(r[1], adds(t, mc.g2)); r[2] = vmax(r[2], adds(t, mc.g3));
    r[3] = vmax(r3, adds(cs, mc.G48));
}

typedef int lds_v4i __attribute__((ext_vector_type(4)));
typedef int vec_v4i __attribute__((ext_vector_type(4)));
struct MultiOut { int mx, act_max8, pas_max8, corner_new; };

template <int KIND, bool TRACE, int SPM = 0, int SL = 16>
__device__ __forceinline__ void multi_rect(const char* table, const FillConsts& fc, const MultiConsts& mc, int l, int (&Ad)[4], int (&Ac)[4],
                                           int (&Pd)[4], int (&Pr)[4], uint2 vb, uint32_t cb_lo, uint32_t cb_hi, int corner, int off_add,
                                           uint32_t* __restrict__ tout, bool store, MultiOut& o, int rz2 = 0, bool fqs_row0 = false, int* zout = nullptr) {
    uint32_t zacc[2] = {0, 0};
    const int offa = splat(off_add);
    int d[4], c[4], pd[4], pr[4];
#pragma unroll
    for (int k = 0; k < 4; k++) {
        d[k] = adds(Ad[k], offa); c[k] = adds(Ac[k], offa); pd[k] = adds(Pd[k], offa); pr[k] = adds(Pr[k], offa);
    }
    o.corner_new = slot_first<SL>(pd[3]) >> 16;
    ScoreKey<KIND> key[4];
#pragma unroll
    for (int k = 0; k < 4; k++) key[k] = make_key<KIND>((int)((vb.x >> (8 * k)) & 0xffu), (int)((vb.y >> (8 * k)) & 0xffu));
    uint32_t kb[4] = {0, 0, 0, 0}, cbs_lo = 0, cbs_hi = 0;
    if constexpr (KIND == KIND_NUC) {
        const uint32_t tb = (uint32_t)(uintptr_t)table;
        const uint32_t k01 = nuc_keys2((uint32_t)__builtin_amdgcn_perm((int)vb.y, (int)vb.x, 0x05010400)), k23 = nuc_keys2((uint32_t)__builtin_amdgcn_perm((int)vb.y, (int)vb.x, 0x07030602));
        kb[0] = add_word(k01, tb, 0); kb[1] = add_word(k01, tb, 1); kb[2] = add_word(k23, tb, 0); kb[3] = add_word(k23, tb, 1);
        cbs_lo = nuc_col_offsets(cb_lo); cbs_hi = nuc_col_offsets(cb_hi);
    }
    int dmax[4] = {0, 0, 0, 0}, tacc[8] = {0, 0, 0, 0, 0, 0, 0, 0};
    int nvD[4] = {0, 0, 0, 0}, nvR[4] = {0, 0, 0, 0};
    int holdD[4] = {0, 0, 0, 0}, holdR[4] = {0, 0, 0, 0};
#pragma unroll
    for (int j = 0; j < STEP; j++) {
        const int cb = (int)(((j < 4 ? cb_lo : cb_hi) >> (8 * (j & 3))) & 0xffu);
        int sc[4];
#pragma unroll
        for (int k = 0; k < 4; k++) {
            if constexpr (KIND == KIND_NUC) sc[k] = lds_read_i32(add_byte(j < 4 ? cbs_lo : cbs_hi, kb[k], j));
            else sc[k] = fetch_score<KIND>(table, key[k], cb);
        }
        int prev = slot_shr1_z<SL>(d[3], l);
        if (j == 0) prev = l == 0 ? (int)((uint32_t)corner << 16) : prev;
        int d00[4];
        d00[0] = __builtin_amdgcn_alignbit(d[3], prev, 16);
#pragma unroll
        for (int k = 1; k < 4; k++) d00[k] = d[k - 1];
        int d11[4], copen[4], cn[4], x[4], r[4];
#pragma unroll
        for (int k = 0; k < 4; k++) {
            d11[k] = adds(d00[k], sc[k]);
            if (SPM == 2 && k == 0) d11[0] = fqs_row0 ? (int)(((uint32_t)d11[0] & 0xffff0000u) | ((uint32_t)rz2 & 0xffffu)) : d11[0];
            if (SPM == 1) d11[k] = vmax(d11[k], rz2);
            copen[k] = adds(d[k], fc.go2);
            cn[k] = vmax(adds(c[k], fc.ge2), copen[k]);
            d11[k] = vmax(d11[k], cn[k]);
            x[k] = adds(d11[k], fc.ome2);
            r[k] = x[k];
        }
        const int r3 = scan_halves(r, fc.ge2, mc);
        const int cs = multi_carry<SL>(r3, mc, l);
        apply_halves(r, r3, cs, fc.ge2, mc);
        int dn[4];
        uint32_t sC[4], sR[4], sCo[4], sRo[4];
#pragma unroll
        for (int k = 0; k < 4; k++) {
            dn[k] = vmax(d11[k], r[k]);
            if (TRACE) {
                sC[k] = (uint32_t)subs(cn[k], dn[k]); sR[k] = (uint32_t)subs(r[k], dn[k]); sCo[k] = (uint32_t)subs(copen[k], cn[k]); sRo[k] = (uint32_t)subs(x[k], r[k]);
            }
            dmax[k] = vmax(dmax[k], dn[k]);
            d[k] = dn[k]; c[k] = cn[k];
        }
        if (TRACE && SPM == 1) {
#pragma unroll
            for (int p2 = 0; p2 < 2; p2++) {
                const uint32_t pZ = (uint32_t)__builtin_amdgcn_perm(subs(rz2, dn[2 * p2 + 1]), subs(rz2, dn[2 * p2]), 0x0b090a08);
                zacc[p2] |= pZ & (0x01010101u << j);
            }
        }
        if (TRACE) {
#pragma unroll
            for (int p2 = 0; p2 < 2; p2++) {
                const uint32_t pC = (uint32_t)__builtin_amdgcn_perm((int)sC[2 * p2 + 1], (int)sC[2 * p2], 0x0b090a08), pR = (uint32_t)__builtin_amdgcn_perm((int)sR[2 * p2 + 1], (int)sR[2 * p2], 0x0b090a08);
                const uint32_t pCo = (uint32_t)__builtin_amdgcn_perm((int)sCo[2 * p2 + 1], (int)sCo[2 * p2], 0x0b090a08), pRo = (uint32_t)__builtin_amdgcn_perm((int)sRo[2 * p2 + 1], (int)sRo[2 * p2], 0x0b090a08);
                const uint32_t lo2 = bfi(0x55555555u, pC, pR), hi2 = bfi(0x55555555u, pCo, pRo);
                const uint32_t nib = bfi(0x33333333u, lo2, hi2);
                if (j & 1) tacc[2 * (j >> 1) + p2] = (int)bfi(0xF0F0F0F0u, nib, (uint32_t)tacc[2 * (j >> 1) + p2]);
                else tacc[2 * (j >> 1) + p2] = (int)nib;
            }
        }
        if (j >= 4) { nvD[j - 4] = __builtin_amdgcn_perm(dn[3], holdD[j - 4], 0x07060302); nvR[j - 4] = __builtin_amdgcn_perm(r[3], holdR[j - 4], 0x07060302); }
        else { holdD[j] = dn[3]; holdR[j] = r[3]; }
    }
    if (TRACE) {
#ifndef MQ_X_NOTRSTORE
        if (store) { *(int4*)tout = int4{tacc[0], tacc[1], tacc[2], tacc[3]}; *(int4*)(tout + 4) = int4{tacc[4], tacc[5], tacc[6], tacc[7]}; }
#else
        asm volatile("" :: "v"(tacc[0]), "v"(tacc[1]), "v"(tacc[2]), "v"(tacc[3]), "v"(tacc[4]), "v"(tacc[5]), "v"(tacc[6]), "v"(tacc[7]));
#endif
    }
#pragma unroll
    for (int k = 0; k < 4; k++) {
        Pd[k] = slot_shl1_keep<SL>(nvD[k], pd[k], l); Pr[k] = slot_shl1_keep<SL>(nvR[k], pr[k], l);
        Ad[k] = d[k]; Ac[k] = c[k];
    }
    {
        const int ma = vmax(vmax(d[0], d[1]), vmax(d[2], d[3])), mb = vmax(vmax(Pd[0], Pd[1]), vmax(Pd[2], Pd[3]));
        const s16x2 sa = as_s(ma), sb = as_s(mb);
        const int xa = vmax(ma, as_i(s16x2{sa.y, sa.x})), xb = vmax(mb, as_i(s16x2{sb.y, sb.x}));
        const s16x2 rr = as_s(slot_first<SL>(__builtin_amdgcn_perm(xb, xa, 0x05040100)));
        o.act_max8 = rr.x; o.pas_max8 = rr.y;
    }
    const int mm = vmax(vmax(dmax[0], dmax[1]), vmax(dmax[2], dmax[3]));
    const int m32 = max(mm & 0xffff, (int)((uint32_t)mm >> 16));
    o.mx = slot_last<SL>(SL == 16 ? wave_prefix_max16(m32) : (SL == 64 ? wave_prefix_max(m32) : wave_prefix_max32(m32)));
    if constexpr (TRACE && SPM == 1) { zout[0] = ~__builtin_amdgcn_perm((int)zacc[1], (int)zacc[0], 0x05040100); zout[1] = ~__builtin_amdgcn_perm((int)zacc[1], (int)zacc[0], 0x07060302); }
}

enum { MR_PAIR = 0, MR_BEST_I, MR_BEST_J, MR_CELLS_LO, MR_CELLS_HI, MR_BUDGET, MR_STATUS, MR_TSLOT, MR_SI, MR_SJ, MR_DIR, MR_PREV_DIR, MR_OFF, MR_OFF_MAX,
       MR_BEST_MAX, MR_Y_DROP, MR_X_ITER, MR_D_CORNER, MR_NSTEPS, MR_TRACE_TOP, MR_NBLOCKS, MR_SEL, MR_WORDS };
__device__ __forceinline__ int mq_load(const char* p) { return __hip_atomic_load((const int*)p, BA_RLX_AGENT); }

#ifndef MQ_PARTIAL_MB
#define MQ_PARTIAL_MB 256
#endif
#ifndef MQ_WAVES_EU
#define MQ_WAVES_EU 4
#endif
template <int PMAX, int KIND, bool TRACE, bool XDROP, int SPM = 0, int MBP = 128, int WPW = WAVES_PER_WG, int EU = MQ_WAVES_EU>
__global__ void __launch_bounds__(WPW * 64, (PMAX >= 16 ? 2 : EU)) k_multi(const BatchParams bp) {
    constexpr uint32_t MB = (uint32_t)MBP;
    constexpr int SL = MBP / 8, NSLOT = 64 / SL;
    constexpr uint32_t ALLM = (1u << NSLOT) - 1u;
    constexpr uint32_t ARR = 2u * MB, BUFL = 4u * ARR, BUFA = BUFL + 64u, SLOTA = 2u * BUFA + 128u;
    static_assert((MBP == 128 || MBP == 256 || MBP == 512) && NSLOT * SLOTA <= MQ_WAVE_BYTES && NSLOT * 2u * BUFL <= MQ_LDS_SCALARS && (MBP == 128 || SPM == 0), "k_multi slot geometry");
    static_assert(MBP != 128 || (BUFA == MQ_BUF_BYTES && SLOTA == MQ_SLOT_BYTES), "ba_params.h");
    constexpr uint32_t MQ_TW = (STEP * MB / 8) * (SPM == 1 ? 2u : 1u);
    constexpr int TB_LB = SPM ? (int)TB_LANE_BYTES_LOC : (int)TB_LANE_BYTES_L2;
    constexpr uint32_t TB_MASK = SPM ? ~0u : (uint32_t)F_CIGAR_EQ;
    extern __shared__ __attribute__((aligned(16))) char smem[];
    const int lane = lane_id(), l = lane & (SL - 1), g = lane / SL;
    const int wave = uni((int)threadIdx.x >> 6);
    {
        char* tab = smem;
        if (KIND == KIND_NUC) {
            nuc_table_fill(tab, bp.matrix, (int)threadIdx.x, WPW * 64);
        } else {
            const int nbytes = KIND == KIND_AA ? 27 * 32 : 2;
            for (int k = (int)threadIdx.x; k < nbytes; k += WPW * 64) tab[k] = (char)bp.matrix[k];
        }
    }
    __syncthreads();
    constexpr uint32_t LCLS = (uint32_t)PMAX * 128u;
    constexpr uint32_t ab = lds_array_bytes_h(LCLS);
    char* base = smem + lds_table_bytes_h(KIND) + (uint32_t)wave * mq_wave_bytes_h(LCLS);
    WaveLds L;
    L.D_col = (short*)(base + 0 * ab); L.C_col = (short*)(base + 1 * ab);
    L.D_row = (short*)(base + 2 * ab); L.R_row = (short*)(base + 3 * ab);
    L.misc = (short*)(base + 4 * ab);
    L.table = smem;
    const int gx = bp.gap_extend;
    const uint32_t stride = bp.tb_stride;
    const bool batch_traceback = TRACE && stride > 0;
#if defined(BA_TIMING) || defined(BA_ENDHIST)
    if (bp.prof && blockIdx.x == 0 && wave == 1 && is_lane(0)) atomicMax(bp.prof + 43, (unsigned long long)__builtin_amdgcn_s_memrealtime());
#endif
#ifdef BA_TIMING
    unsigned long long t_solo = 0, t_quad = 0, t_wait = 0, n_solo = 0, n_quad = 0;
#endif
    if (batch_traceback && wave == 0 && blockIdx.x % stride == 0) {
        if (!(bp.flags & 0x800u))
        traceback_consumer<TB_LB, 8, 3, true>(bp, TB_MASK, (unsigned char*)base, 64u, true, 1);
#if defined(BA_TIMING) || defined(BA_ENDHIST)
        if (bp.prof && is_lane(0)) atomicMax(bp.prof + 42, (unsigned long long)__builtin_amdgcn_s_memrealtime());
#endif
        return;
    }
    const uint32_t cons_before = batch_traceback ? (blockIdx.x + stride - 1) / stride + (blockIdx.x % stride == 0 ? 1u : 0u) : 0u;
    const uint32_t fill_wave = blockIdx.x * WPW + (uint32_t)wave - cons_before;
    const uint32_t max_size = bp.max_size;
    const bool keep_pre = XDROP || MB < max_size;
    char* const wave_mem = (char*)bp.big + (uint64_t)fill_wave * MQ_WAVE_BYTES;

    auto coldp_big = [&]() { const __attribute__((address_space(4))) BatchParams* p = (const __attribute__((address_space(4))) BatchParams*)__builtin_amdgcn_kernarg_segment_ptr(); asm volatile("" : "+s"(p)); return p->big; };
    auto fill_wave_of = [&]() { uint32_t b = blockIdx.x, w = (uint32_t)wave; asm volatile("" : "+s"(b), "+s"(w)); const uint32_t st = ((const __attribute__((address_space(4))) BatchParams*)__builtin_amdgcn_kernarg_segment_ptr())->tb_stride;
                                const uint32_t cb = (TRACE && st > 0) ? (b + st - 1) / st + (b % st == 0 ? 1u : 0u) : 0u; return b * WPW + w - cb; };
    uint32_t live_m = 0, pend_m = 0;
    uint32_t w_next = 0, w_end = 0;
    bool more = true, drain = false, fin_counted = false;
#define don_final (bp.mq_donate + gridDim.x * WPW)
#define don_offers (don_final + 32)
    auto slot_mem_of = [&](uint32_t id, uint32_t s_i) {
        const uint32_t db = id / WPW;
        const uint32_t dcb = batch_traceback ? (db + stride - 1) / stride + (db % stride == 0 ? 1u : 0u) : 0u;
        return (char*)bp.big + (uint64_t)(id - dcb) * MQ_WAVE_BYTES + s_i * SLOTA;
    };
    auto claim_offer = [&](uint32_t my_id, uint32_t& id_out, int& s_out) {
        uint32_t avail = 0;
        if (is_lane(0)) avail = __hip_atomic_load(don_offers, BA_RLX_AGENT);
        if ((int)uni((int)avail) <= 0) return false;
        const uint32_t n_ids = gridDim.x * WPW;
        for (uint32_t k0 = 0; k0 < n_ids; k0 += 64) {
            const uint32_t idx = ((my_id & ~63u) + k0 + (uint32_t)lane) % n_ids;
            const uint32_t v = __hip_atomic_load(bp.mq_donate + idx, BA_RLX_AGENT) & ALLM;
            unsigned long long m = __ballot(v != 0u);
            while (m) {
                const int src = __builtin_ctzll(m);
                const uint32_t vv = (uint32_t)__builtin_amdgcn_readlane((int)v, src), id = (uint32_t)__builtin_amdgcn_readlane((int)idx, src);
                const int s_i = __builtin_ctz(vv);
                uint32_t old = 0;
                if (is_lane(0)) {
                    old = __hip_atomic_fetch_and(bp.mq_donate + id, ~(1u << s_i), BA_RLX_AGENT);
                    if ((old >> s_i) & 1u) __hip_atomic_fetch_sub(don_offers, 1u, BA_RLX_AGENT);
                }
                old = (uint32_t)uni((int)old);
                if ((old >> s_i) & 1u) { id_out = id; s_out = s_i; return true; }
                m &= m - 1;
            }
        }
        return false;
    };
    auto try_refill = [&](uint32_t my_id) {
        uint32_t id = 0; int s_o = 0;
        if ((bp.flags & 0x1000u) || !claim_offer(my_id, id, s_o)) return false;
        __builtin_amdgcn_fence(__ATOMIC_ACQUIRE, "agent");
        const int e = __builtin_ctz(~live_m & ALLM);
        const char* src = slot_mem_of(id, (uint32_t)s_o);
        char* dst = wave_mem + (uint32_t)e * SLOTA;
#pragma unroll
        for (int k = 0; k < (int)(SLOTA / 256u); k++) *(int*)(dst + 256 * k + 4 * lane) = mq_load(src + 256 * k + 4 * lane);
        asm volatile("s_waitcnt vmcnt(0)" ::: "memory");
        live_m |= 1u << e;
        return true;
    };
    auto my_id_of = [&]() { uint32_t b = blockIdx.x, w = (uint32_t)wave; asm volatile("" : "+s"(b), "+s"(w)); return b * WPW + w; };

    for (;;) {
        for (;;) {
            int solo = -1; bool fresh = false, to_end = false;
            uint32_t new_pair = 0, donor_id = ~0u;
            if (pend_m) solo = __builtin_ctz(pend_m);
            else if (more && (drain ? live_m == 0u : live_m != ALLM)) {
                if (w_next == w_end) {
                    uint32_t v = 0;
                    if (is_lane(0)) v = atomicAdd(bp.work_counter, bp.work_chunk);
                    w_next = (uint32_t)uni((int)v);
                    if (w_next >= bp.n) { more = false; w_next = w_end = 0; continue; }
                    w_end = min(w_next + bp.work_chunk, bp.n);
                }
                new_pair = w_next++; solo = __builtin_ctz(~live_m & ALLM); fresh = true;
                to_end = drain;
                if (new_pair + bp.mq_drain >= bp.n) drain = true;
            } else if (live_m && live_m != ALLM && MB < (uint32_t)(MQ_PARTIAL_MB)) {
                solo = __builtin_ctz(live_m); to_end = true;
                if (TRACE && bp.mq_donate) {
                    const uint32_t my_id = my_id_of();
                    uint32_t don = 0;
                    if (is_lane(0)) don = __hip_atomic_load(bp.mq_donate + my_id, BA_RLX_AGENT);
                    don = (uint32_t)uni((int)don) >> 8;
                    if (!(don & 1u)) {
                        if (try_refill(my_id)) continue;
                        const uint32_t others = live_m & ~(1u << solo);
                        if (others) {
                            __builtin_amdgcn_fence(__ATOMIC_RELEASE, "agent");
                            asm volatile("s_waitcnt vmcnt(0)" ::: "memory");
                        }
                        if (is_lane(0)) {
                            __hip_atomic_store(bp.mq_donate + my_id, others | 0x100u | (others ? 0x200u : 0u), BA_RLX_AGENT);
                            if (others) __hip_atomic_fetch_add(don_offers, (uint32_t)__builtin_popcount(others), BA_RLX_AGENT);
                        }
                        asm volatile("s_waitcnt vmcnt(0)" ::: "memory");
                        if (is_lane(0)) __hip_atomic_fetch_add(don_final, 1u, BA_RLX_AGENT);
                    } else if (don & 2u) {
                        uint32_t old = 0;
                        if (is_lane(0)) {
                            old = __hip_atomic_fetch_and(bp.mq_donate + my_id, ~(1u << solo), BA_RLX_AGENT);
                            if ((old >> solo) & 1u) __hip_atomic_fetch_sub(don_offers, 1u, BA_RLX_AGENT);
                        }
                        old = (uint32_t)uni((int)old);
                        if (!((old >> solo) & 1u)) { live_m &= ~(1u << solo); continue; }
                    }
                }
            } else if (TRACE && bp.mq_donate && !live_m && !more) {
                const uint32_t my_id = my_id_of();
                if (is_lane(0) && !(__hip_atomic_fetch_or(bp.mq_donate + my_id, 0x100u, BA_RLX_AGENT) & 0x100u)) __hip_atomic_fetch_add(don_final, 1u, BA_RLX_AGENT);
                const uint32_t n_fill = gridDim.x * WPW - (batch_traceback ? (gridDim.x + stride - 1) / stride : 0u);
                bool got = false;
                uint32_t nap = 1;
                for (;;) {
                    uint32_t nf = 0;
                    if (is_lane(0)) nf = __hip_atomic_load(don_final, BA_RLX_AGENT);
                    nf = (uint32_t)uni((int)nf);
                    got = !(bp.flags & 0x2000u) && claim_offer(my_id, donor_id, solo);
                    if (got || nf >= n_fill) break;
                    for (uint32_t z = 0; z < nap; z++) __builtin_amdgcn_s_sleep(127);
                    nap = nap < 16u ? nap * 2u : 16u;
                }
                if (!got) { donor_id = ~0u; break; }
                __builtin_amdgcn_fence(__ATOMIC_ACQUIRE, "agent");
                to_end = true;
            }
            else {
                if constexpr (TRACE && MB >= (uint32_t)(MQ_PARTIAL_MB)) {
                    if (bp.mq_donate && live_m && live_m != ALLM && !more && !fin_counted) {
                        fin_counted = true;
                        const uint32_t my_id = my_id_of();
                        if (is_lane(0) && !(__hip_atomic_fetch_or(bp.mq_donate + my_id, 0x100u, BA_RLX_AGENT) & 0x100u)) __hip_atomic_fetch_add(don_final, 1u, BA_RLX_AGENT);
                    }
                }
                break;
            }

            BA_TSTAMP(ts_a);
            const FillConsts fc = make_fill_consts(lane, bp.gap_open, gx);
            Aligner<PMAX, KIND, TRACE, XDROP, SPM != 0, true, MBP> al(bp, L, fc);
            PairState st{};
            uint32_t s_pair, s_slot;
            char* smem_s = wave_mem + (uint32_t)solo * SLOTA;
            if (donor_id != ~0u) smem_s = slot_mem_of(donor_id, (uint32_t)solo);
            char* const rec = smem_s + 2 * BUFA;
            al.ckpt = bp.ckpt + (uint64_t)(fill_wave + bp.ckpt_wave0) * 8 * bp.max_size;
            if (fresh) {
                s_pair = new_pair;
                s_slot = fill_wave * bp.slots_per_wave;
                if (batch_traceback) {
                    BA_TSTAMP(tw_a);
                    uint32_t seen = 0, idle_n = 0;
                    for (;;) {
                        uint32_t f = 0, head = 0;
                        if ((uint32_t)lane < bp.slots_per_wave) f = __hip_atomic_load(bp.slot_free + s_slot + lane, BA_RLX_AGENT);
                        if (is_lane(0)) head = __hip_atomic_load(bp.tb_ctrl + 32, BA_RLX_AGENT);
                        const unsigned long long fm = __ballot(f != 0);
                        if (fm) {
                            s_slot += (uint32_t)__builtin_ctzll(fm);
                            if (is_lane(0)) __hip_atomic_store(bp.slot_free + s_slot, 0u, BA_RLX_AGENT);
                            break;
                        }
                        head = (uint32_t)uni((int)head);
                        if (head != seen) { seen = head; idle_n = 0; }
                        else if ((++idle_n & 2047u) == 0 && traceback_help_one<TB_LB, true>(bp, TB_MASK, (unsigned char*)base)) idle_n = 0;
                        __builtin_amdgcn_s_sleep(64);
                    }
#ifdef BA_TIMING
                    t_wait += __builtin_amdgcn_s_memtime() - tw_a;
#endif
                } else if (TRACE) {
                    s_slot += (uint32_t)solo;
                }
            } else {
                const int rv = lane < MR_WORDS ? mq_load(rec + 4 * lane) : 0;
#define BA_W(v, k) __builtin_amdgcn_readlane(v, k)
                const uint32_t s_sel = (uint32_t)BA_W(rv, MR_SEL);
                const char* live_b = smem_s + (s_sel ^ 1u) * BUFA; const char* ck_b = smem_s + s_sel * BUFA;
                const int cv = lane < 16 ? mq_load(ck_b + BUFL + 4 * lane) : 0;
                s_pair = (uint32_t)BA_W(rv, MR_PAIR); s_slot = (uint32_t)BA_W(rv, MR_TSLOT);
                st.si = (uint32_t)BA_W(rv, MR_SI); st.sj = (uint32_t)BA_W(rv, MR_SJ); st.dir = BA_W(rv, MR_DIR); st.prev_dir = BA_W(rv, MR_PREV_DIR);
                st.off = BA_W(rv, MR_OFF); st.off_max = BA_W(rv, MR_OFF_MAX); st.best_max = BA_W(rv, MR_BEST_MAX);
                st.y_drop_iter = (uint32_t)BA_W(rv, MR_Y_DROP); st.x_drop_iter = BA_W(rv, MR_X_ITER); st.D_corner = BA_W(rv, MR_D_CORNER);
                st.trace_top = (uint32_t)BA_W(rv, MR_TRACE_TOP); st.nblocks = (uint32_t)BA_W(rv, MR_NBLOCKS);
                const uint32_t ns = (uint32_t)BA_W(rv, MR_NSTEPS);
                st.best_i = (uint32_t)BA_W(rv, MR_BEST_I); st.best_j = (uint32_t)BA_W(rv, MR_BEST_J);
                st.cells = ((unsigned long long)(uint32_t)BA_W(rv, MR_CELLS_LO) | ((unsigned long long)(uint32_t)BA_W(rv, MR_CELLS_HI) << 32)) + (unsigned long long)ns * (STEP * MB);
                const uint32_t bud = (uint32_t)BA_W(rv, MR_BUDGET);
                st.step_budget = bud > ns ? bud - ns : 1u;
                st.status = (uint32_t)BA_W(rv, MR_STATUS);
                const int flag = BA_W(cv, 0);
                const bool ck_pre = flag != 0;
                st.ck_i = (uint32_t)BA_W(cv, 1); st.ck_j = (uint32_t)BA_W(cv, 2); st.ck_off = BA_W(cv, 3);
                st.ck_tt = (uint32_t)BA_W(cv, 4) + (flag ? MQ_TW : 0u); st.ck_nb = (uint32_t)BA_W(cv, 5) + (flag ? 1u : 0u);
                const int ck_dir = BA_W(cv, 6), ck_offadd = BA_W(cv, 7), ck_corner = BA_W(cv, 8);
#undef BA_W
                {
                    int reg[16], ckr[16];
                    const bool lr = st.dir == DIR_RIGHT, cr = ck_dir == DIR_RIGHT;
                    const uint32_t oAd = (lr ? 0u : 2 * ARR) + l * 16, oAc = (lr ? ARR : 3 * ARR) + l * 16, oPd = (lr ? 2 * ARR : 0u) + l * 16, oPr = (lr ? 3 * ARR : ARR) + l * 16;
                    const uint32_t cAd = (cr ? 0u : 2 * ARR) + l * 16, cAc = (cr ? ARR : 3 * ARR) + l * 16, cPd = (cr ? 2 * ARR : 0u) + l * 16, cPr = (cr ? 3 * ARR : ARR) + l * 16;
#pragma unroll
                    for (int k = 0; k < 4; k++) {
                        reg[k] = mq_load(live_b + oAd + 4 * k); reg[4 + k] = mq_load(live_b + oAc + 4 * k); reg[8 + k] = mq_load(live_b + oPd + 4 * k); reg[12 + k] = mq_load(live_b + oPr + 4 * k);
                        ckr[k] = mq_load(ck_b + cAd + 4 * k); ckr[4 + k] = mq_load(ck_b + cAc + 4 * k); ckr[8 + k] = mq_load(ck_b + cPd + 4 * k); ckr[12 + k] = mq_load(ck_b + cPr + 4 * k);
                    }
                    al.import_slot(reg, ckr, s_pair, ck_pre || MB < max_size, ck_pre, ck_dir, ck_offadd, ck_corner, st.ck_i, st.ck_j, st.best_i, st.best_j, st.ck_off);
                }
            }
            al.trace = bp.trace_arena + (uint64_t)s_slot * bp.trace_stride;
            al.blocks = bp.blocks + (uint64_t)s_slot * bp.blocks_stride;
            int keepv = 0;
            park<0>(keepv, (int)live_m); park<1>(keepv, (int)pend_m); park<2>(keepv, (int)w_next); park<3>(keepv, (int)w_end);
            park<4>(keepv, (more ? 1 : 0) | (fresh ? 2 : 0) | (to_end ? 4 : 0) | (drain ? 8 : 0)); park<5>(keepv, solo); park<6>(keepv, (int)s_pair); park<7>(keepv, (int)s_slot);
            BA_TSTAMP(tr_a);
            __builtin_amdgcn_s_setprio(MQ_SOLO_PRIO);
            st = al.run(s_pair, s_slot, batch_traceback, nullptr, fresh ? MM_FRESH : MM_RESUME, st, !to_end, !fresh && !to_end);
            __builtin_amdgcn_s_setprio(0);
            live_m = (uint32_t)unpark<0>(keepv); pend_m = (uint32_t)unpark<1>(keepv); w_next = (uint32_t)unpark<2>(keepv); w_end = (uint32_t)unpark<3>(keepv);
            { const int fl = unpark<4>(keepv); more = fl & 1; fresh = fl & 2; to_end = fl & 4; drain = fl & 8; }
            solo = unpark<5>(keepv); s_pair = (uint32_t)unpark<6>(keepv); s_slot = (uint32_t)unpark<7>(keepv);
            char* const smem_s2 = (char*)coldp_big() + (uint64_t)fill_wave_of() * MQ_WAVE_BYTES + (uint32_t)solo * SLOTA;
            char* const rec2 = smem_s2 + 2 * BUFA;
#ifdef BA_TIMING
            {
                const unsigned long long tr_b = __builtin_amdgcn_s_memtime();
                al.prof[45] += tr_b - tr_a; al.prof[46] += fresh ? 1 : 0;
                if (bp.prof && is_lane(0)) {
                    for (int k = 0; k < 48; k++) if (k != 17 && !(k >= 20 && k < 32) && !(k >= 40 && k < 44)) atomicAdd(bp.prof + k, al.prof[k]);
                    atomicAdd(bp.prof + (fresh ? 56 : (to_end ? 58 : 57)), tr_b - tr_a);
                }
            }
#endif
            pend_m &= ~(1u << solo);
            if (st.exited) {
                const bool rgt = st.dir == DIR_RIGHT;
                if (lane < SL) {
                    const int l8 = 8 * l;
                    const int4 a_d = *(const int4*)((rgt ? L.D_col : L.D_row) + l8), a_c = *(const int4*)((rgt ? L.C_col : L.R_row) + l8);
                    const int4 p_d = *(const int4*)((rgt ? L.D_row : L.D_col) + l8), p_r = *(const int4*)((rgt ? L.R_row : L.C_col) + l8);
                    char* b1 = smem_s2 + BUFA;
                    *(int4*)(b1 + l * 16) = a_d; *(int4*)(b1 + ARR + l * 16) = a_c; *(int4*)(b1 + 2 * ARR + l * 16) = p_d; *(int4*)(b1 + 3 * ARR + l * 16) = p_r;
                    if (MB < max_size) {
                        char* b0 = smem_s2;
                        *(int4*)(b0 + l * 16) = *(const int4*)(L.D_col + MB + l8); *(int4*)(b0 + ARR + l * 16) = *(const int4*)(L.C_col + MB + l8);
                        *(int4*)(b0 + 2 * ARR + l * 16) = *(const int4*)(L.D_row + MB + l8); *(int4*)(b0 + 3 * ARR + l * 16) = *(const int4*)(L.R_row + MB + l8);
                    }
                }
                if (is_lane(0)) {
                    char* b0 = smem_s2;
                    *(int4*)(b0 + BUFL) = int4{0, (int)st.ck_i, (int)st.ck_j, st.ck_off}; *(int4*)(b0 + BUFL + 16) = int4{(int)st.ck_tt, (int)st.ck_nb, DIR_RIGHT, 0};
                    *(int*)(b0 + BUFL + 32) = 0;
                    int* rc = (int*)rec2;
                    rc[MR_PAIR] = (int)s_pair; rc[MR_BEST_I] = (int)st.best_i; rc[MR_BEST_J] = (int)st.best_j; rc[MR_CELLS_LO] = (int)(uint32_t)st.cells; rc[MR_CELLS_HI] = (int)(uint32_t)(st.cells >> 32);
                    rc[MR_BUDGET] = (int)st.step_budget; rc[MR_STATUS] = (int)st.status; rc[MR_TSLOT] = (int)s_slot; rc[MR_SI] = (int)st.si; rc[MR_SJ] = (int)st.sj; rc[MR_DIR] = st.dir;
                    rc[MR_PREV_DIR] = st.prev_dir; rc[MR_OFF] = st.off; rc[MR_OFF_MAX] = st.off_max; rc[MR_BEST_MAX] = st.best_max; rc[MR_Y_DROP] = (int)st.y_drop_iter;
                    rc[MR_X_ITER] = st.x_drop_iter; rc[MR_D_CORNER] = st.D_corner; rc[MR_NSTEPS] = 0; rc[MR_TRACE_TOP] = (int)st.trace_top; rc[MR_NBLOCKS] = (int)st.nblocks; rc[MR_SEL] = 0;
                }
                lds_sync();
                live_m |= 1u << solo;
            } else live_m &= ~(1u << solo);
#ifdef BA_TIMING
            t_solo += __builtin_amdgcn_s_memtime() - ts_a; n_solo++;
#endif
        }
        if (!live_m) break;

        {
            BA_TSTAMP(tq_a);
            char* const slot_mem = wave_mem + (uint32_t)g * SLOTA;
            const int x_drop = bp.x_drop;
            FillConsts fq;
            fq.go2 = splat(bp.gap_open); fq.ge2 = splat(gx); fq.ome2 = splat(clamp16(bp.gap_open - gx));
            MultiConsts mc = make_multi_consts(l, gx);
            const uint64_t tcap64 = bp.trace_stride, bcap64 = bp.blocks_stride;
            const uint32_t tcap = (uint32_t)(tcap64 < 0x7fffffffull ? tcap64 : 0x7fffffffull), bcap = (uint32_t)(bcap64 < 0x7fffffffull ? bcap64 : 0x7fffffffull);
            const bool live = (live_m >> g) & 1u;
            const char* rec = slot_mem + 2 * BUFA;
#define BA_R(k) (live ? mq_load(rec + 4 * (k)) : 0)
            const uint32_t pair = (uint32_t)BA_R(MR_PAIR), tslot = (uint32_t)BA_R(MR_TSLOT);
            uint32_t si = (uint32_t)BA_R(MR_SI), sj = (uint32_t)BA_R(MR_SJ), y_drop = (uint32_t)BA_R(MR_Y_DROP);
            uint32_t nblocks = (uint32_t)BA_R(MR_NBLOCKS), sel = (uint32_t)BA_R(MR_SEL);
            const uint32_t tt_in = (uint32_t)BA_R(MR_TRACE_TOP), tt0 = tt_in - nblocks * MQ_TW;
            int dir = BA_R(MR_DIR), prev_dir = BA_R(MR_PREV_DIR), off = BA_R(MR_OFF), off_max = BA_R(MR_OFF_MAX), best_max = BA_R(MR_BEST_MAX);
            int x_iter = BA_R(MR_X_ITER), D_corner = BA_R(MR_D_CORNER);
#undef BA_R
            int A_d[4], A_c[4], P_d[4], P_r[4];
            {
                const char* b = slot_mem + (sel ^ 1u) * BUFA + l * 16;
#pragma unroll
                for (int k = 0; k < 4; k++) {
                    A_d[k] = live ? mq_load(b + 4 * k) : 0; A_c[k] = live ? mq_load(b + ARR + 4 * k) : 0;
                    P_d[k] = live ? mq_load(b + 2 * ARR + 4 * k) : 0; P_r[k] = live ? mq_load(b + 3 * ARR + 4 * k) : 0;
                }
                cells_split(A_d); cells_split(A_c); cells_split(P_d); cells_split(P_r);
            }
            char* const lbuf = base + (uint32_t)g * (2u * BUFL);
            constexpr uint32_t MQ_LSC_STATE = 9u, MQ_LSC_PAIR = 20u;
            static_assert(2u * MQ_LSC_STATE <= MQ_LSC_PAIR && MQ_LSC_PAIR + 12u <= MQ_LSC_INTS && (4u * MQ_LSC_PAIR) % 16u == 0 && (4u * MQ_LSC_INTS) % 16u == 0, "a slot's scalars in LDS");
            int* const lsc = (int*)(base + MQ_LDS_SCALARS) + (uint32_t)g * MQ_LSC_INTS;
            lds_sync();
            const unsigned long long qa_r = TRACE ? 0ull : (unsigned long long)(bp.pool + (live ? bp.q_off[pair] : 0ull)), ra_r = TRACE ? 0ull : (unsigned long long)(bp.pool + (live ? bp.r_off[pair] : 0ull));
            const uint32_t qlen_r = (!TRACE && live) ? bp.q_len[pair] : 0u, rlen_r = (!TRACE && live) ? bp.r_len[pair] : 0u;
            if (TRACE && l == 0) {
                const unsigned long long qo = live ? bp.q_off[pair] : 0ull, ro = live ? bp.r_off[pair] : 0ull;
                *(int4*)(lsc + MQ_LSC_PAIR) = int4{(int)(uint32_t)qo, (int)(uint32_t)(qo >> 32), (int)(uint32_t)ro, (int)(uint32_t)(ro >> 32)};
                const long long room = (long long)tcap - (long long)(MQ_TW + 64u) - (long long)tt_in;
                const unsigned long long nb_room = room < 0 ? 0ull : (unsigned long long)nblocks + (unsigned long long)room / MQ_TW + 1ull;
                const uint32_t nb_lim = (uint32_t)(nb_room < (unsigned long long)bcap ? nb_room : (unsigned long long)bcap);
                *(int4*)(lsc + MQ_LSC_PAIR + 4) = int4{live ? (int)bp.q_len[pair] : 0, live ? (int)bp.r_len[pair] : 0, (int)nb_lim, 0};
                const unsigned long long ta = (unsigned long long)(bp.trace_arena + (uint64_t)tslot * bp.trace_stride), ba = (unsigned long long)(bp.blocks + (uint64_t)tslot * bp.blocks_stride);
                *(int4*)(lsc + MQ_LSC_PAIR + 8) = int4{(int)(uint32_t)ta, (int)(uint32_t)(ta >> 32), (int)(uint32_t)ba, (int)(uint32_t)(ba >> 32)};
            }
            if (live) {
                const char* cb = slot_mem + sel * BUFA;
                char* d = lbuf + sel * BUFL + l * 16;
#pragma unroll
                for (int a = 0; a < 4; a++) {
                    const char* sp = cb + a * ARR + l * 16;
                    *(int4*)(d + a * ARR) = cells_split(int4{mq_load(sp), mq_load(sp + 4), mq_load(sp + 8), mq_load(sp + 12)});
                }
                if ((uint32_t)l < MQ_LSC_STATE) lsc[sel * MQ_LSC_STATE + l] = mq_load(cb + BUFL + 4 * l);
            }
            lds_sync();
            uint2 pf_qv = {0, 0}, pf_rv = {0, 0}, pf_qc = {0, 0}, pf_rc = {0, 0}; bool pf_ok = false;
            bool leave = false;
            auto stage = [&](uint32_t lb, uint32_t ls, uint32_t which, uint32_t s_i, uint32_t s_j, int s_off, uint32_t s_tt, uint32_t s_nb, int s_dir, int s_offadd, int s_corner) {
                typedef __attribute__((address_space(3))) lds_v4i* lds_int4_ptr;
                typedef __attribute__((address_space(3))) int* lds_int_ptr;
                const lds_int4_ptr b = (lds_int4_ptr)(uintptr_t)(lb + which * BUFL);
                b[0] = lds_v4i{A_d[0], A_d[1], A_d[2], A_d[3]}; b[ARR / 16] = lds_v4i{A_c[0], A_c[1], A_c[2], A_c[3]};
                b[2 * ARR / 16] = lds_v4i{P_d[0], P_d[1], P_d[2], P_d[3]}; b[3 * ARR / 16] = lds_v4i{P_r[0], P_r[1], P_r[2], P_r[3]};
                if (l == 0) {
                    const lds_int_ptr sc = (lds_int_ptr)(uintptr_t)ls + which * MQ_LSC_STATE;
                    sc[0] = 1; sc[1] = (int)s_i; sc[2] = (int)s_j; sc[3] = s_off; sc[4] = (int)s_tt; sc[5] = (int)s_nb; sc[6] = s_dir; sc[7] = s_offadd; sc[8] = s_corner;
                }
            };
            const uint32_t base32 = (uint32_t)(uintptr_t)base;
            typedef const __attribute__((address_space(1))) uint8_t* glb_cu8_ptr;
            typedef const __attribute__((address_space(1))) uint32_t* glb_cu32_ptr;
            do {
                const bool right = dir == DIR_RIGHT;
                uint32_t lid;
                asm volatile("v_mbcnt_lo_u32_b32 %0, -1, 0\n\tv_mbcnt_hi_u32_b32 %0, -1, %0" : "=v"(lid));
                const uint32_t l8 = (lid & (uint32_t)(SL - 1)) * 8u;
                const uint32_t lbuf_s = base32 + (lid / (uint32_t)SL) * (2u * BUFL) + 2u * l8;
                const uint32_t lsc_s = base32 + (uint32_t)MQ_LDS_SCALARS + (lid / (uint32_t)SL) * (4u * (uint32_t)MQ_LSC_INTS);
                const __attribute__((address_space(4))) BatchParams* kargs = (const __attribute__((address_space(4))) BatchParams*)__builtin_amdgcn_kernarg_segment_ptr();
                asm volatile("" : "+s"(kargs));
                const glb_cu8_ptr pool_g = (glb_cu8_ptr)kargs->pool;
                const bool pool64 = TRACE && (kargs->flags & (uint32_t)F_POOL64);
                int4 cA = {0, 0, 0, 0}, cB = {0, 0, 0, 0}, cC = {0, 0, 0, 0};
                if (TRACE) {
                    typedef const __attribute__((address_space(3))) lds_v4i* lds_cint4_ptr;
                    const lds_v4i a4 = *(lds_cint4_ptr)(uintptr_t)(lsc_s + 4u * MQ_LSC_PAIR), b4 = *(lds_cint4_ptr)(uintptr_t)(lsc_s + 4u * (MQ_LSC_PAIR + 4u)),
                                  c4 = *(lds_cint4_ptr)(uintptr_t)(lsc_s + 4u * (MQ_LSC_PAIR + 8u));
                    cA = int4{a4.x, a4.y, a4.z, a4.w}; cB = int4{b4.x, b4.y, b4.z, b4.w}; cC = int4{c4.x, c4.y, c4.z, c4.w};
                }
                const uint8_t* const qp = (const uint8_t*)qa_r; const uint8_t* const rp = (const uint8_t*)ra_r;
                const uint32_t qo32 = (uint32_t)cA.x, ro32 = (uint32_t)cA.z;
                const uint32_t qlen = TRACE ? (uint32_t)cB.x : qlen_r, rlen = TRACE ? (uint32_t)cB.y : rlen_r;
                const uint32_t ri = right ? si : sj, rj = (right ? sj : si) + (MB - STEP);
                const uint32_t lenV = right ? qlen : rlen, lenC = right ? rlen : qlen;
                const bool q_out = si + MB > qlen, r_out = sj + MB > rlen;
                bool elig = XDROP || ri + MB <= lenV || rj + STEP <= lenC;
                const uint32_t trace_top = tt0 + nblocks * MQ_TW;
                if (TRACE) elig = elig && nblocks < (uint32_t)cB.z;
                leave = live && !elig;
                const bool run = live && !leave;
                const int off_n = off_max;
                const int off_add = sat16(off - off_n);
                const int corner = (prev_dir != dir && prev_dir != DIR_GROW) ? sat16(D_corner + off_add) : 0;
#ifndef MQ_X_NOSTAGE
                if (live) stage(lbuf_s, lsc_s, sel ^ 1u, si, sj, off_n, trace_top, nblocks, dir, off_add, corner);
#endif
                asm volatile("" : "+v"(mc.laneKG), "+v"(mc.lanem1KG), "+v"(mc.w0));
                uint2 vb, cbv;
                {
                    const uint8_t* Vp = right ? qp : rp; const uint8_t* Cp = right ? rp : qp;
                    vb = right ? pf_qv : pf_rv; cbv = right ? pf_rc : pf_qc;
                    if (__any(run && !pf_ok)) {
                        if (run && !pf_ok) {
                            if constexpr (TRACE) {
                                const unsigned long long vo = right ? ((unsigned long long)(uint32_t)cA.x | ((unsigned long long)(uint32_t)cA.y << 32)) : ((unsigned long long)(uint32_t)cA.z | ((unsigned long long)(uint32_t)cA.w << 32));
                                const unsigned long long co = right ? ((unsigned long long)(uint32_t)cA.z | ((unsigned long long)(uint32_t)cA.w << 32)) : ((unsigned long long)(uint32_t)cA.x | ((unsigned long long)(uint32_t)cA.y << 32));
                                const glb_cu32_ptr vp = (glb_cu32_ptr)(pool_g + (vo + (ri + l8))), cp = (glb_cu32_ptr)(pool_g + (co + rj));
                                vb.x = vp[0]; vb.y = vp[1]; cbv.x = cp[0]; cbv.y = cp[1];
                            } else {
                            const uint32_t* vp = (const uint32_t*)(Vp + (ri + l8));
                            vb.x = vp[0]; vb.y = vp[1];
                            const uint32_t* cp = (const uint32_t*)(Cp + rj);
                            cbv.x = cp[0]; cbv.y = cp[1];
                            }
                        }
                    }
                    asm volatile("" : "+v"(vb.x), "+v"(vb.y));
                    if (!pool64) if (run) {
                        if constexpr (TRACE) {
                            const glb_cu32_ptr a = (glb_cu32_ptr)(pool_g + (unsigned long long)(qo32 + (si + l8))), b = (glb_cu32_ptr)(pool_g + (unsigned long long)(ro32 + (sj + l8)));
                            const glb_cu32_ptr cq = (glb_cu32_ptr)(pool_g + (unsigned long long)(qo32 + si) + MB), cr = (glb_cu32_ptr)(pool_g + (unsigned long long)(ro32 + sj) + MB);
                            pf_qv.x = a[0]; pf_qv.y = a[1]; pf_rv.x = b[0]; pf_rv.y = b[1];
                            pf_qc.x = cq[0]; pf_qc.y = cq[1]; pf_rc.x = cr[0]; pf_rc.y = cr[1];
                        } else {
                        const uint32_t* a = (const uint32_t*)(qp + (si + l8)); const uint32_t* b = (const uint32_t*)(rp + (sj + l8));
                        const uint32_t* cq = (const uint32_t*)(qp + si + MB); const uint32_t* cr = (const uint32_t*)(rp + sj + MB);
                        pf_qv.x = a[0]; pf_qv.y = a[1]; pf_rv.x = b[0]; pf_rv.y = b[1];
                        pf_qc.x = cq[0]; pf_qc.y = cq[1]; pf_rc.x = cr[0]; pf_rc.y = cr[1];
                        }
                        pf_ok = true;
                    }
                }
                uint32_t* tw = nullptr;
                if (TRACE) {
                    typedef __attribute__((address_space(1))) uint32_t* glb_u32_ptr;
                    tw = (uint32_t*)(glb_u32_ptr)((unsigned long long)(uint32_t)cC.x | ((unsigned long long)(uint32_t)cC.y << 32)) + (trace_top + l8);
                    if (run && l == 0) {
                        static_assert(sizeof(BlockRec) == 16, "a record as four words");
                        const uint32_t hw = right ? ((uint32_t)MB | ((uint32_t)STEP << 16)) : ((uint32_t)STEP | ((uint32_t)MB << 16));
                        typedef __attribute__((address_space(1))) vec_v4i* glb_rec_ptr;
                        ((glb_rec_ptr)((unsigned long long)(uint32_t)cC.z | ((unsigned long long)(uint32_t)cC.w << 32)))[nblocks] =
                            vec_v4i{(int)((right ? ri : rj) | 0x80000000u) , (int)(right ? rj : ri), (int)hw, (int)(trace_top | (right ? 0x80000000u : 0u))};
                    }
                }
                MultiOut o;
                int zw[2] = {0, 0};
                multi_rect<KIND, TRACE, SPM, SL>(smem, fq, mc, l, A_d, A_c, P_d, P_r, vb, cbv.x, cbv.y, corner, off_add, tw, run, o, SPM ? splat(sat16(ZERO - off_n)) : 0,
                                             SPM == 2 && right && ri == 0u && l == 0, zw);
                if (TRACE && SPM == 1 && run) *(int2*)(tw - 8 * l + 128 + 2 * l) = int2{zw[0], zw[1]};

                const int right_max = right ? o.act_max8 : o.pas_max8, down_max = right ? o.pas_max8 : o.act_max8;
                const int new_off_max = off_n + o.mx - ZERO;
                const bool improve = new_off_max > best_max;
                const uint32_t new_y = improve ? 0u : y_drop + 1;
                bool stop = q_out && r_out;
                if (XDROP) stop = stop || (!improve && new_off_max < best_max - x_drop && x_iter >= 1);
                stop = stop || (!q_out && !r_out && 2 * MB <= max_size && new_y > MB / STEP - 1);
                const bool commit = run && !stop;
                leave = leave || (run && stop);
                {
                    const bool imp = commit && improve;
                    if (keep_pre) sel ^= imp ? 1u : 0u;
                    best_max = imp ? new_off_max : best_max;
                    off = commit ? off_n : off; off_max = commit ? new_off_max : off_max; y_drop = commit ? new_y : y_drop;
                    prev_dir = commit ? dir : prev_dir; D_corner = commit ? o.corner_new : D_corner;
                    if (TRACE) nblocks += commit ? 1u : 0u;
                    if (XDROP) x_iter = commit ? ((new_off_max < best_max - x_drop) ? x_iter + 1 : 0) : x_iter;
                    const bool go_down = r_out || (!q_out && down_max > right_max);
                    si += (commit && go_down) ? (uint32_t)STEP : 0u; sj += (commit && !go_down) ? (uint32_t)STEP : 0u;
                    const int ndir = go_down ? DIR_DOWN : DIR_RIGHT;
                    const unsigned long long swap_m = __ballot(ndir != dir);
#pragma unroll
                    for (int k = 0; k < 4; k++) {
                        const int td = A_d[k], tc = A_c[k];
                        A_d[k] = sel_mask(swap_m, P_d[k], td); A_c[k] = sel_mask(swap_m, P_r[k], tc); P_d[k] = sel_mask(swap_m, td, P_d[k]); P_r[k] = sel_mask(swap_m, tc, P_r[k]);
                    }
                    dir = commit ? ndir : dir;
                }
#ifdef BA_TIMING
                n_quad++;
#endif
            } while (!__any(leave));
            const uint32_t trace_top = tt0 + nblocks * MQ_TW;
            if (live && !leave) stage((uint32_t)(uintptr_t)(lbuf + l * 16), (uint32_t)(uintptr_t)lsc, sel ^ 1u, si, sj, 0, trace_top, nblocks, dir, 0, 0);
            lds_sync();
            if (live) {
#pragma unroll
                for (int w = 0; w < 2; w++) {
                    const char* sp = lbuf + w * BUFL + l * 16;
                    char* d = slot_mem + w * BUFA + l * 16;
#pragma unroll
                    for (int a = 0; a < 4; a++) *(int4*)(d + a * ARR) = cells_join(*(const int4*)(sp + a * ARR));
                    if ((uint32_t)l < MQ_LSC_STATE) *(int*)(slot_mem + w * BUFA + BUFL + 4 * l) = lsc[w * MQ_LSC_STATE + l];
                }
            }
            lds_sync();
            if (live && l == 0) {
                int* rc = (int*)(slot_mem + 2 * BUFA);
                const uint32_t nsteps = (uint32_t)mq_load((const char*)(rc + MR_NSTEPS)) + ((si + sj) - (uint32_t)mq_load((const char*)(rc + MR_SI)) - (uint32_t)mq_load((const char*)(rc + MR_SJ))) / (uint32_t)STEP;
                rc[MR_SI] = (int)si; rc[MR_SJ] = (int)sj; rc[MR_DIR] = dir; rc[MR_PREV_DIR] = prev_dir; rc[MR_OFF] = off; rc[MR_OFF_MAX] = off_max; rc[MR_BEST_MAX] = best_max;
                rc[MR_Y_DROP] = (int)y_drop; rc[MR_X_ITER] = x_iter; rc[MR_D_CORNER] = D_corner; rc[MR_NSTEPS] = (int)nsteps; rc[MR_TRACE_TOP] = (int)trace_top;
                rc[MR_NBLOCKS] = (int)nblocks; rc[MR_SEL] = (int)sel;
            }
            const unsigned long long lm = __ballot(leave && l == 0);
            pend_m = 0;
#pragma unroll
            for (int sl_i = 0; sl_i < NSLOT; sl_i++) pend_m |= (uint32_t)((lm >> (sl_i * SL)) & 1ull) << sl_i;
#ifdef BA_TIMING
            t_quad += __builtin_amdgcn_s_memtime() - tq_a;
#endif
        }
    }
#ifdef BA_TIMING
    if (bp.prof && is_lane(0)) {
        atomicMax(bp.prof + 40, (unsigned long long)__builtin_amdgcn_s_memrealtime());
        atomicAdd(bp.prof + 50, t_solo); atomicAdd(bp.prof + 51, t_quad); atomicAdd(bp.prof + 52, t_wait); atomicAdd(bp.prof + 53, n_solo); atomicAdd(bp.prof + 54, n_quad); atomicAdd(bp.prof + 55, 1ull);
    }
#endif
#ifdef BA_ENDHIST
    if (bp.prof && is_lane(0)) {
        const unsigned long long t0 = __hip_atomic_load(bp.prof + 43, BA_RLX_AGENT), t = __builtin_amdgcn_s_memrealtime();
        const unsigned long long k = t0 && t > t0 ? (t - t0) / 400000ull : 0ull;
        atomicAdd(bp.prof + 64 + (k < 63ull ? k : 63ull), 1ull);
        atomicMax(bp.prof + 40, t);
    }
#endif
    if (batch_traceback) {
        lds_sync();
#ifndef MQ_HELPER_LANES
#define MQ_HELPER_LANES 0u
#endif
        if constexpr (SPM != 0) traceback_consumer<TB_LB, TB_CELLS_PER_STEP, BA_RING_DEPTH, true>(bp, TB_MASK, (unsigned char*)base, 4u, false);
        else {
#if MQ_HELPER_LANES == 0
        traceback_helper_wave<true, true>(bp, (uint32_t*)base, 2048u);
#else
        traceback_consumer<(int)TB_LANE_BYTES_L2, TB_CELLS_PER_STEP, BA_RING_DEPTH, true>(bp, (uint32_t)F_CIGAR_EQ, (unsigned char*)base, MQ_HELPER_LANES, false);
#endif
        }
#if defined(BA_TIMING) || defined(BA_ENDHIST)
        if (bp.prof && is_lane(0)) atomicMax(bp.prof + 41, (unsigned long long)__builtin_amdgcn_s_memrealtime());
#endif
    }
}

#undef don_final
#undef don_offers
}
```

block_aligner_amd/csrc/ba_params.h:

```cpp
#pragma once
#include <stdint.h>

namespace ba {

constexpr int ZERO = 1 << 14;
constexpr int STEP = 8;
constexpr int KIND_AA = 0, KIND_NUC = 1, KIND_BYTES = 2, KIND_PROFILE = 3;
constexpr int DIR_RIGHT = 0, DIR_DOWN = 1, DIR_GROW = 2;

enum : uint32_t {
    F_TRACE = 1u << 0, F_XDROP = 1u << 1, F_LOCAL = 1u << 2, F_FQS = 1u << 3, F_FQE = 1u << 4, F_CIGAR_EQ = 1u << 5,
    F_POOL64 = 1u << 15,
    F_PAD_NEG = 1u << 14
};
enum : uint32_t { ST_OK = 0, ST_TRACE_OVERFLOW = 1, ST_BLOCKS_OVERFLOW = 2, ST_CIGAR_OVERFLOW = 4, ST_TRACEBACK_LOST = 8, ST_WATCHDOG = 16, ST_SLOT_TIMEOUT = 32, ST_MODE = 64,
                  ST_CLASS_OVERFLOW = 128  };

struct BlockRec {
    uint32_t i, j;
    uint16_t h, w;
    uint32_t trace_base;
};

struct SlotInfo { uint32_t pair, nblocks, end_i, end_j; };

#if defined(__HIPCC__)
#define BA_HD __host__ __device__
#else
#define BA_HD
#endif
BA_HD inline uint32_t profile_positions(uint32_t len, uint32_t max_size) { return (len + max_size + 17u) & ~1u; }
BA_HD inline uint64_t profile_image_bytes(uint32_t len, uint32_t max_size) { return (uint64_t)profile_positions(len, max_size) * (32 + 64 + 6); }

struct PairCont {
    uint32_t pair, si, sj; int32_t dir, prev_dir, off, off_max, best_max;
    uint32_t y_drop_iter; int32_t x_drop_iter, D_corner; uint32_t best_i, best_j, ck_i, ck_j; int32_t ck_off;
    unsigned long long cells; uint32_t step_budget;
    uint32_t trace_top, nblocks, ck_trace_top, ck_nblocks, status;
    uint32_t borders[4][16];
    uint32_t ckpt[4][16];
};
static_assert(sizeof(PairCont) == 96 + 512, "PairCont layout");

struct BatchParams {
    const uint8_t* pool;
    const uint64_t* q_off; const uint32_t* q_len;
    const uint64_t* r_off; const uint32_t* r_len;
    uint32_t n;
    int32_t gap_open, gap_extend;
    uint32_t min_size, max_size;
    int32_t x_drop;
    uint32_t flags;
    const int8_t* matrix;
    int32_t* score; uint32_t* query_idx; uint32_t* reference_idx;
    uint32_t* cig_ops; const uint64_t* cig_off; uint32_t* cig_start; uint32_t* cig_len;
    unsigned long long* cells;
    uint32_t* status;
    uint32_t* nblocks_out;
    uint32_t* slot_out;
    uint32_t* trace_words_out;
    uint32_t* trace_arena; uint64_t trace_stride;
    BlockRec* blocks; uint64_t blocks_stride;
    const uint64_t* trace_off; const uint64_t* blocks_off;
    short* ckpt;
    short* big;
    uint32_t* work_counter;
    unsigned long long* prof;
    uint32_t tb_stride;
    uint32_t slots_per_wave;
    uint32_t n_slots;
    uint32_t tb_reserve;
    uint32_t tb_qmask;
    uint32_t* tb_queue;
    uint32_t* tb_ctrl;
    uint32_t* slot_free;
    SlotInfo* slot_info;
    uint32_t cont_mode;
    const PairCont* cont_in; const uint32_t* cont_in_flag;
    PairCont* cont_out; uint32_t* cont_out_flag;
    uint32_t* cq_queue;
    uint32_t* cq_ctrl;
    uint32_t cq_producers;
    uint32_t cq_side;
    uint32_t inline_len2;
    uint32_t ckpt_wave0;
    uint32_t mq_drain;
    uint32_t* mq_donate;
    uint32_t mq_waves;
    uint32_t walk_wave_n;
    uint32_t work_chunk;
    uint32_t sm_excl_first;
    uint32_t sm_excl_n;
    uint32_t tb_i, tb_j, tb_nblocks, tb_slot;
};


constexpr uint32_t BIG_TILE = 2048;
BA_HD constexpr uint64_t big_array_shorts(uint32_t max_size) { return (uint64_t)max_size + 64; }
BA_HD constexpr uint64_t big_wave_shorts(uint32_t max_size) { return 8 * big_array_shorts(max_size); }

constexpr uint32_t MQ_B_HOST = 128;
constexpr uint32_t MQ_BUF_BYTES = 4 * 256 + 64, MQ_SLOT_BYTES = 2 * MQ_BUF_BYTES + 128, MQ_WAVE_BYTES = 4 * MQ_SLOT_BYTES;
constexpr uint32_t MQ_LDS_SCALARS = 8192, MQ_LSC_INTS = 32, MQ_LDS_BYTES = 8192 + 4 * MQ_LSC_INTS * 4;
constexpr uint32_t SM_B_HOST = 32, SM_SLOTS = 16;
constexpr uint32_t SM_BUF_BYTES = 4 * 64 + 32, SM_SLOT_BYTES = 2 * SM_BUF_BYTES + 128, SM_WAVE_BYTES = SM_SLOTS * SM_SLOT_BYTES;
constexpr uint32_t SM_LDS_SCALARS = 8192, SM_LDS_BYTES = 8192 + SM_SLOTS * 2 * 32;
#ifndef BA_WAVES_PER_WG
#define BA_WAVES_PER_WG 8
#endif
constexpr int WAVES_PER_WG = BA_WAVES_PER_WG;
constexpr int MQ_GEOM_WPW = 4;

BA_HD constexpr uint32_t lds_array_bytes_h(uint32_t max_size) { return max_size * 2 + 32; }
BA_HD constexpr uint32_t lds_wave_bytes_h(uint32_t max_size) { return 4 * lds_array_bytes_h(max_size) + 128; }
BA_HD constexpr uint32_t lds_table_bytes_h(int kind) { return kind == KIND_NUC ? 8192 : 896; }
BA_HD constexpr uint32_t lds_wg_bytes_h(int kind, uint32_t max_size) { return lds_table_bytes_h(kind) + WAVES_PER_WG * lds_wave_bytes_h(max_size); }
BA_HD constexpr uint32_t mq_wave_bytes_h(uint32_t max_size) { return lds_wave_bytes_h(max_size) > MQ_LDS_BYTES ? lds_wave_bytes_h(max_size) : MQ_LDS_BYTES; }
BA_HD constexpr uint32_t mq_wg_bytes_h(int kind, uint32_t max_size, uint32_t wpw = WAVES_PER_WG) { return lds_table_bytes_h(kind) + wpw * mq_wave_bytes_h(max_size); }
constexpr uint32_t SM_PROF_STAGE = 16 * 256;
BA_HD constexpr uint32_t sm_wave_bytes_h(uint32_t max_size, int kind = 0) {
    return (lds_wave_bytes_h(max_size) > SM_LDS_BYTES ? lds_wave_bytes_h(max_size) : SM_LDS_BYTES) + (kind == KIND_PROFILE ? SM_PROF_STAGE : 0u);
}
BA_HD constexpr uint32_t sm_wg_bytes_h(int kind, uint32_t max_size) { return lds_table_bytes_h(kind) + WAVES_PER_WG * sm_wave_bytes_h(max_size, kind); }
constexpr uint32_t TB_LANE_BYTES = 76, TB_LUT_BYTES = 128, TB_LDS_BYTES = 5120;
constexpr uint32_t TB_LANE_BYTES_L2 = 100;
constexpr uint32_t TB_LANE_BYTES_LOC = 116, TB_LDS_BYTES_LOC = 7680;
static_assert(TB_LUT_BYTES + 64 * TB_LANE_BYTES_LOC <= TB_LDS_BYTES_LOC, "k_walk LDS (LOCAL_START)");
constexpr uint32_t TB_LDS_BYTES_L2 = 6784;
static_assert(TB_LUT_BYTES + 64 * TB_LANE_BYTES_L2 <= TB_LDS_BYTES_L2, "k_walk LDS (slot rectangles)");
static_assert(MQ_LDS_BYTES % 16 == 0 && TB_LUT_BYTES + 64 * TB_LANE_BYTES_L2 <= MQ_LDS_BYTES, "k_multi LDS");
constexpr uint32_t TB_DIAG_LUT_L2 = 256, TB_DIAG_LUT_STD = 64;
static_assert(TB_LUT_BYTES + 64 * TB_LANE_BYTES + TB_DIAG_LUT_STD <= TB_LDS_BYTES && TB_LUT_BYTES + TB_LANE_BYTES + 8 + TB_DIAG_LUT_STD <= lds_wave_bytes_h(128), "traceback LDS regions");
static_assert((TB_LUT_BYTES + 64 * TB_LANE_BYTES) % 8 == 0 && (TB_LUT_BYTES + 64 * TB_LANE_BYTES_L2) % 8 == 0, "tb_diag's tables are read 8 bytes at a time");
static_assert(TB_LUT_BYTES + 64 * TB_LANE_BYTES_L2 + TB_DIAG_LUT_L2 <= TB_LDS_BYTES_L2 && TB_LUT_BYTES + 64 * TB_LANE_BYTES_L2 + TB_DIAG_LUT_L2 <= MQ_LDS_BYTES, "tb_diag's tables (slot rectangles)");
static_assert(TB_LUT_BYTES + 64 * TB_LANE_BYTES_LOC <= MQ_LDS_BYTES && TB_LUT_BYTES + 64 * TB_LANE_BYTES_LOC <= SM_LDS_BYTES, "special-mode walk records in a wave's region");

}
```

Before: 2665.

## Specialize multi-slot kernel for 64-bit pools and restructure step loop eligibility

Adds a separate k_multi_p64 instantiation selected on the host when the sequence pool exceeds 32-bit offsets, so the common kernel drops the runtime pool64 branches. The inner step loop is restructured: eligibility is checked up front and after each step, trace words are kept in registers and stored once per committed step, and dead slots write to scratch slot memory instead of being guarded per store. It also adds an optional step-count profiling flag. This cuts per-step predication and branches in the hot loop, at the cost of more kernel variants and more complex control flow.

```diff
diff --git a/block_aligner_amd/csrc/ba_host.cpp b/block_aligner_amd/csrc/ba_host.cpp
--- a/block_aligner_amd/csrc/ba_host.cpp
+++ b/block_aligner_amd/csrc/ba_host.cpp
@@ -240,13 +240,14 @@
     bool pad_negative = false;
     bool handle_mode = false;
     DevBuf hblk, rblk;
+    bool pool64() const { return (uint64_t)pool.bytes + 2ull * max_size + 8ull > 0xffffffffull || dev_env("BA_POOL64"); }
     BatchParams params() const {
         BatchParams bp{};
         bp.pool = pool.as<uint8_t>();
         bp.q_off = q_off.as<uint64_t>(); bp.q_len = q_len.as<uint32_t>();
         bp.r_off = r_off.as<uint64_t>(); bp.r_len = r_len.as<uint32_t>();
         bp.n = n; bp.gap_open = gap_open; bp.gap_extend = gap_extend;
-        bp.min_size = min_size; bp.max_size = max_size; bp.x_drop = x_drop; bp.flags = mode | (dev_env("BA_NO_FAST") ? 0x100u : 0u) | ((dev_env("BA_SKIP_WALK") || dev_env("BA_NO_TRACEBACK")) ? 0x200u : 0u) | ((handle_mode || dev_env("BA_NO_SPEC")) ? 0x400u : 0u) | (dev_env("BA_NO_TB_WAVES") ? 0x800u : 0u) | (dev_env("BA_NO_REFILL") ? 0x1000u : 0u) | (dev_env("BA_NO_STEAL") ? 0x2000u : 0u) | ((pad_negative && !dev_env("BA_NO_END_CLIP")) ? (uint32_t)ba::F_PAD_NEG : 0u) | (((uint64_t)pool.bytes + 2ull * max_size + 8ull > 0xffffffffull || dev_env("BA_POOL64")) ? (uint32_t)ba::F_POOL64 : 0u);
+        bp.min_size = min_size; bp.max_size = max_size; bp.x_drop = x_drop; bp.flags = mode | (dev_env("BA_NO_FAST") ? 0x100u : 0u) | ((dev_env("BA_SKIP_WALK") || dev_env("BA_NO_TRACEBACK")) ? 0x200u : 0u) | ((handle_mode || dev_env("BA_NO_SPEC")) ? 0x400u : 0u) | (dev_env("BA_NO_TB_WAVES") ? 0x800u : 0u) | (dev_env("BA_NO_REFILL") ? 0x1000u : 0u) | (dev_env("BA_NO_STEAL") ? 0x2000u : 0u) | ((pad_negative && !dev_env("BA_NO_END_CLIP")) ? (uint32_t)ba::F_PAD_NEG : 0u) | (pool64() ? (uint32_t)ba::F_POOL64 : 0u) | (dev_env("BA_COUNT_STEPS") ? (uint32_t)ba::F_COUNT_STEPS : 0u);
         bp.matrix = matrix.as<int8_t>();
         bp.score = score.as<int32_t>(); bp.query_idx = qidx.as<uint32_t>(); bp.reference_idx = ridx.as<uint32_t>();
         bp.cig_ops = ((mode & BA_TRACE) && !handle_mode && !dev_env("BA_NO_TRACEBACK")) ? cig_ops.as<uint32_t>() : nullptr;
@@ -544,7 +545,11 @@
     default: return ba::MQ_WAVE_BYTES;
     }
 }
-static const void* kernel_fn(const BaBatch* b, const ba::KernelEntry* k, bool trace, int form) { return k->fn[form][trace][(b->mode & BA_X_DROP) != 0]; }
+static const void* kernel_fn(const BaBatch* b, const ba::KernelEntry* k, bool trace, int form) {
+    const int xd = (b->mode & BA_X_DROP) != 0;
+    if (trace && k->fn64[form][xd] && b->pool64()) return k->fn64[form][xd];
+    return k->fn[form][trace][xd];
+}
 static hipError_t kernel_lds_opt_in(const void* fn, unsigned lds) {
     return lds > 64 * 1024 ? hipFuncSetAttribute(fn, hipFuncAttributeMaxDynamicSharedMemorySize, (int)lds) : hipSuccess;
 }
diff --git a/block_aligner_amd/csrc/ba_kernels.hip b/block_aligner_amd/csrc/ba_kernels.hip
--- a/block_aligner_amd/csrc/ba_kernels.hip
+++ b/block_aligner_amd/csrc/ba_kernels.hip
@@ -34,36 +34,45 @@
 #define K_SMALL_S1(T, X) ba::k_small<BA_PMAX, BA_KIND, T, X, 1>
 #define K_SMALL_S2(T, X) ba::k_small<BA_PMAX, BA_KIND, T, X, 2>
 #define K_QUAD(T, X) ba::k_quad<BA_KIND, T, X>
+#define P_MULTI(X) ba::k_multi_p64<BA_PMAX, BA_KIND, X>
+#define P_MULTI_256(X) ba::k_multi_p64<BA_PMAX, BA_KIND, X, 0, 256>
+#define P_MULTI_512(X) ba::k_multi_p64<BA_PMAX, BA_KIND, X, 0, 512>
+#define P_MULTI_G2(X) ba::k_multi_p64<BA_PMAX, BA_KIND, X, 0, 128, ba::MQ_GEOM_WPW, 2>
+#define P_MULTI_G3(X) ba::k_multi_p64<BA_PMAX, BA_KIND, X, 0, 128, ba::MQ_GEOM_WPW, 3>
+#define P_MULTI_S1(X) ba::k_multi_p64<BA_PMAX, BA_KIND, X, 1>
+#define P_MULTI_S2(X) ba::k_multi_p64<BA_PMAX, BA_KIND, X, 2>
 #define BA_TX(K) {{(const void*)K(false, false), (const void*)K(false, true)}, {(const void*)K(true, false), (const void*)K(true, true)}}
-#define BA_ENTRY(FAM, WPW, K) {FAM, WPW, 0u, {BA_TX(K), {}}}
-#define BA_ENTRY_SPM(FAM, WPW, K1, K2) {FAM, WPW, 0u, {BA_TX(K1), BA_TX(K2)}}
+#define BA_PX(P) {(const void*)P(false), (const void*)P(true)}
+#define BA_ENTRY(FAM, WPW, K) {FAM, WPW, 0u, {BA_TX(K), {}}, {}}
+#define BA_ENTRY_P64(FAM, WPW, K, P) {FAM, WPW, 0u, {BA_TX(K), {}}, {BA_PX(P), {}}}
+#define BA_ENTRY_SPM(FAM, WPW, K1, K2, P1, P2) {FAM, WPW, 0u, {BA_TX(K1), BA_TX(K2)}, {BA_PX(P1), BA_PX(P2)}}
 
 static const ba::KernelEntry g_entries[] = {
     BA_ENTRY(BA_BIG ? ba::FAM_TILED : ba::FAM_PAIR, ba::WAVES_PER_WG, K_ALIGN),
 #if BA_KIND != 3 && !BA_SPECIAL && !BA_BIG
-    BA_ENTRY(ba::FAM_MULTI, ba::WAVES_PER_WG, K_MULTI),
+    BA_ENTRY_P64(ba::FAM_MULTI, ba::WAVES_PER_WG, K_MULTI, P_MULTI),
 #if BA_KIND == 1 && BA_PMAX >= 4
-    BA_ENTRY(ba::FAM_MULTI_256, ba::WAVES_PER_WG, K_MULTI_256),
+    BA_ENTRY_P64(ba::FAM_MULTI_256, ba::WAVES_PER_WG, K_MULTI_256, P_MULTI_256),
 #endif
 #if BA_KIND == 1 && BA_PMAX >= 8
-    BA_ENTRY(ba::FAM_MULTI_512, ba::WAVES_PER_WG, K_MULTI_512),
+    BA_ENTRY_P64(ba::FAM_MULTI_512, ba::WAVES_PER_WG, K_MULTI_512, P_MULTI_512),
 #endif
 #if BA_KIND == 1 && (BA_PMAX == 4 || BA_PMAX == 8)
-    BA_ENTRY(ba::FAM_MULTI_G3, ba::MQ_GEOM_WPW, K_MULTI_G3),
-    BA_ENTRY(ba::FAM_MULTI_G2, ba::MQ_GEOM_WPW, K_MULTI_G2),
+    BA_ENTRY_P64(ba::FAM_MULTI_G3, ba::MQ_GEOM_WPW, K_MULTI_G3, P_MULTI_G3),
+    BA_ENTRY_P64(ba::FAM_MULTI_G2, ba::MQ_GEOM_WPW, K_MULTI_G2, P_MULTI_G2),
 #endif
 #endif
 #if !BA_SPECIAL && !BA_BIG && BA_PMAX <= 8
     BA_ENTRY(ba::FAM_SMALL, ba::WAVES_PER_WG, K_SMALL),
 #endif
 #if BA_SPECIAL && !BA_BIG && BA_KIND != 3
-    BA_ENTRY_SPM(ba::FAM_MULTI, ba::WAVES_PER_WG, K_MULTI_S1, K_MULTI_S2),
+    BA_ENTRY_SPM(ba::FAM_MULTI, ba::WAVES_PER_WG, K_MULTI_S1, K_MULTI_S2, P_MULTI_S1, P_MULTI_S2),
 #endif
 #if BA_SPECIAL && !BA_BIG && BA_PMAX <= 8 && BA_KIND != 3
-    BA_ENTRY_SPM(ba::FAM_SMALL, ba::WAVES_PER_WG, K_SMALL_S1, K_SMALL_S2),
+    {ba::FAM_SMALL, ba::WAVES_PER_WG, 0u, {BA_TX(K_SMALL_S1), BA_TX(K_SMALL_S2)}, {}},
 #endif
 #if BA_PMAX == 1 && !BA_SPECIAL && !BA_BIG
-    {ba::FAM_QUAD, ba::WAVES_PER_WG, ba::lds_table_bytes_h(BA_KIND) + ba::WAVES_PER_WG * 4 * ba::QUAD_SLOT_BYTES, {BA_TX(K_QUAD), {}}},
+    {ba::FAM_QUAD, ba::WAVES_PER_WG, ba::lds_table_bytes_h(BA_KIND) + ba::WAVES_PER_WG * 4 * ba::QUAD_SLOT_BYTES, {BA_TX(K_QUAD), {}}, {}},
 #endif
 };
 [[maybe_unused]] static const int g_registered = ba::register_kernels(BA_KIND, BA_PMAX, BA_SPECIAL != 0, g_entries, (int)(sizeof g_entries / sizeof g_entries[0]));
diff --git a/block_aligner_amd/csrc/ba_launch.h b/block_aligner_amd/csrc/ba_launch.h
--- a/block_aligner_amd/csrc/ba_launch.h
+++ b/block_aligner_amd/csrc/ba_launch.h
@@ -28,6 +28,7 @@
     unsigned wpw;
     unsigned lds;
     const void* fn[2][2][2];
+    const void* fn64[2][2];
 };
 
 int register_kernels(int kind, int pmax, bool special, const KernelEntry* entries, int n);
diff --git a/block_aligner_amd/csrc/ba_multi.hpp b/block_aligner_amd/csrc/ba_multi.hpp
--- a/block_aligner_amd/csrc/ba_multi.hpp
+++ b/block_aligner_amd/csrc/ba_multi.hpp
@@ -18,15 +18,15 @@
     return r;
 }
 
-template <int SL> __device__ __forceinline__ int slot_first(int v) {
+template <int SL> __device__ __forceinline__ int slot_first(int v, int wl) {
     if constexpr (SL == 16) return row_bcast<0>(v);
     else if constexpr (SL == 64) return __builtin_amdgcn_readfirstlane(v);
-    else return __builtin_amdgcn_ds_bpermute((lane_id() & 32) << 2, v);
-}
-template <int SL> __device__ __forceinline__ int slot_last(int v) {
+    else return __builtin_amdgcn_ds_bpermute((wl & 32) << 2, v);
+}
+template <int SL> __device__ __forceinline__ int slot_last(int v, int wl) {
     if constexpr (SL == 16) return row_bcast<15>(v);
     else if constexpr (SL == 64) return __builtin_amdgcn_readlane(v, 63);
-    else return __builtin_amdgcn_ds_bpermute(((lane_id() & 32) + 31) << 2, v);
+    else return __builtin_amdgcn_ds_bpermute(((wl & 32) + 31) << 2, v);
 }
 template <int SL> __device__ __forceinline__ int slot_shr1_z(int v, int l) {
     if constexpr (SL == 16) return row_shr1_z(v);
@@ -105,7 +105,7 @@
 template <int KIND, bool TRACE, int SPM = 0, int SL = 16>
 __device__ __forceinline__ void multi_rect(const char* table, const FillConsts& fc, const MultiConsts& mc, int l, int (&Ad)[4], int (&Ac)[4],
                                            int (&Pd)[4], int (&Pr)[4], uint2 vb, uint32_t cb_lo, uint32_t cb_hi, int corner, int off_add,
-                                           uint32_t* __restrict__ tout, bool store, MultiOut& o, int rz2 = 0, bool fqs_row0 = false, int* zout = nullptr) {
+                                           int (&tout)[8], MultiOut& o, int wl, int rz2 = 0, bool fqs_row0 = false, int* zout = nullptr) {
     uint32_t zacc[2] = {0, 0};
     const int offa = splat(off_add);
     int d[4], c[4], pd[4], pr[4];
@@ -113,7 +113,7 @@
     for (int k = 0; k < 4; k++) {
         d[k] = adds(Ad[k], offa); c[k] = adds(Ac[k], offa); pd[k] = adds(Pd[k], offa); pr[k] = adds(Pr[k], offa);
     }
-    o.corner_new = slot_first<SL>(pd[3]) >> 16;
+    o.corner_new = slot_first<SL>(pd[3], wl) >> 16;
     ScoreKey<KIND> key[4];
 #pragma unroll
     for (int k = 0; k < 4; k++) key[k] = make_key<KIND>((int)((vb.x >> (8 * k)) & 0xffu), (int)((vb.y >> (8 * k)) & 0xffu));
@@ -190,11 +190,8 @@
         else { holdD[j] = dn[3]; holdR[j] = r[3]; }
     }
     if (TRACE) {
-#ifndef MQ_X_NOTRSTORE
-        if (store) { *(int4*)tout = int4{tacc[0], tacc[1], tacc[2], tacc[3]}; *(int4*)(tout + 4) = int4{tacc[4], tacc[5], tacc[6], tacc[7]}; }
-#else
-        asm volatile("" :: "v"(tacc[0]), "v"(tacc[1]), "v"(tacc[2]), "v"(tacc[3]), "v"(tacc[4]), "v"(tacc[5]), "v"(tacc[6]), "v"(tacc[7]));
-#endif
+#pragma unroll
+        for (int k = 0; k < 8; k++) tout[k] = tacc[k];
     }
 #pragma unroll
     for (int k = 0; k < 4; k++) {
@@ -205,12 +202,12 @@
         const int ma = vmax(vmax(d[0], d[1]), vmax(d[2], d[3])), mb = vmax(vmax(Pd[0], Pd[1]), vmax(Pd[2], Pd[3]));
         const s16x2 sa = as_s(ma), sb = as_s(mb);
         const int xa = vmax(ma, as_i(s16x2{sa.y, sa.x})), xb = vmax(mb, as_i(s16x2{sb.y, sb.x}));
-        const s16x2 rr = as_s(slot_first<SL>(__builtin_amdgcn_perm(xb, xa, 0x05040100)));
+        const s16x2 rr = as_s(slot_first<SL>(__builtin_amdgcn_perm(xb, xa, 0x05040100), wl));
         o.act_max8 = rr.x; o.pas_max8 = rr.y;
     }
     const int mm = vmax(vmax(dmax[0], dmax[1]), vmax(dmax[2], dmax[3]));
     const int m32 = max(mm & 0xffff, (int)((uint32_t)mm >> 16));
-    o.mx = slot_last<SL>(SL == 16 ? wave_prefix_max16(m32) : (SL == 64 ? wave_prefix_max(m32) : wave_prefix_max32(m32)));
+    o.mx = slot_last<SL>(SL == 16 ? wave_prefix_max16(m32) : (SL == 64 ? wave_prefix_max(m32) : wave_prefix_max32(m32)), wl);
     if constexpr (TRACE && SPM == 1) { zout[0] = ~__builtin_amdgcn_perm((int)zacc[1], (int)zacc[0], 0x05040100); zout[1] = ~__builtin_amdgcn_perm((int)zacc[1], (int)zacc[0], 0x07060302); }
 }
 
@@ -224,8 +221,8 @@
 #ifndef MQ_WAVES_EU
 #define MQ_WAVES_EU 4
 #endif
-template <int PMAX, int KIND, bool TRACE, bool XDROP, int SPM = 0, int MBP = 128, int WPW = WAVES_PER_WG, int EU = MQ_WAVES_EU>
-__global__ void __launch_bounds__(WPW * 64, (PMAX >= 16 ? 2 : EU)) k_multi(const BatchParams bp) {
+template <int PMAX, int KIND, bool TRACE, bool XDROP, int SPM, int MBP, int WPW, int EU, bool P64>
+__device__ __forceinline__ void multi_body(const BatchParams& bp) {
     constexpr uint32_t MB = (uint32_t)MBP;
     constexpr int SL = MBP / 8, NSLOT = 64 / SL;
     constexpr uint32_t ALLM = (1u << NSLOT) - 1u;
@@ -581,7 +578,9 @@
                 const unsigned long long nb_room = room < 0 ? 0ull : (unsigned long long)nblocks + (unsigned long long)room / MQ_TW + 1ull;
                 const uint32_t nb_lim = (uint32_t)(nb_room < (unsigned long long)bcap ? nb_room : (unsigned long long)bcap);
                 *(int4*)(lsc + MQ_LSC_PAIR + 4) = int4{live ? (int)bp.q_len[pair] : 0, live ? (int)bp.r_len[pair] : 0, (int)nb_lim, 0};
-                const unsigned long long ta = (unsigned long long)(bp.trace_arena + (uint64_t)tslot * bp.trace_stride), ba = (unsigned long long)(bp.blocks + (uint64_t)tslot * bp.blocks_stride);
+                static_assert(4u * MB + (SPM == 1 ? MB : 0u) <= BUFA && sizeof(BlockRec) <= BUFA, "a dead slot's stores stay inside its own buffers");
+                const unsigned long long ta = live ? (unsigned long long)(bp.trace_arena + (uint64_t)tslot * bp.trace_stride) : (unsigned long long)slot_mem;
+                const unsigned long long ba = live ? (unsigned long long)(bp.blocks + (uint64_t)tslot * bp.blocks_stride) : (unsigned long long)(slot_mem + BUFA);
                 *(int4*)(lsc + MQ_LSC_PAIR + 8) = int4{(int)(uint32_t)ta, (int)(uint32_t)(ta >> 32), (int)(uint32_t)ba, (int)(uint32_t)(ba >> 32)};
             }
             if (live) {
@@ -595,15 +594,15 @@
                 if ((uint32_t)l < MQ_LSC_STATE) lsc[sel * MQ_LSC_STATE + l] = mq_load(cb + BUFL + 4 * l);
             }
             lds_sync();
-            uint2 pf_qv = {0, 0}, pf_rv = {0, 0}, pf_qc = {0, 0}, pf_rc = {0, 0}; bool pf_ok = false;
-            bool leave = false;
+            uint2 pf_qv = {0, 0}, pf_rv = {0, 0}, pf_qc = {0, 0}, pf_rc = {0, 0};
+            bool leave = false, rolled = false;
             auto stage = [&](uint32_t lb, uint32_t ls, uint32_t which, uint32_t s_i, uint32_t s_j, int s_off, uint32_t s_tt, uint32_t s_nb, int s_dir, int s_offadd, int s_corner) {
                 typedef __attribute__((address_space(3))) lds_v4i* lds_int4_ptr;
                 typedef __attribute__((address_space(3))) int* lds_int_ptr;
                 const lds_int4_ptr b = (lds_int4_ptr)(uintptr_t)(lb + which * BUFL);
                 b[0] = lds_v4i{A_d[0], A_d[1], A_d[2], A_d[3]}; b[ARR / 16] = lds_v4i{A_c[0], A_c[1], A_c[2], A_c[3]};
                 b[2 * ARR / 16] = lds_v4i{P_d[0], P_d[1], P_d[2], P_d[3]}; b[3 * ARR / 16] = lds_v4i{P_r[0], P_r[1], P_r[2], P_r[3]};
-                if (l == 0) {
+                {
                     const lds_int_ptr sc = (lds_int_ptr)(uintptr_t)ls + which * MQ_LSC_STATE;
                     sc[0] = 1; sc[1] = (int)s_i; sc[2] = (int)s_j; sc[3] = s_off; sc[4] = (int)s_tt; sc[5] = (int)s_nb; sc[6] = s_dir; sc[7] = s_offadd; sc[8] = s_corner;
                 }
@@ -611,7 +610,52 @@
             const uint32_t base32 = (uint32_t)(uintptr_t)base;
             typedef const __attribute__((address_space(1))) uint8_t* glb_cu8_ptr;
             typedef const __attribute__((address_space(1))) uint32_t* glb_cu32_ptr;
+            auto eligible = [&](uint32_t s_i, uint32_t s_j, int s_dir, uint32_t s_nb, uint32_t qlen, uint32_t rlen, uint32_t nb_lim) {
+                const bool rt = s_dir == DIR_RIGHT;
+                bool e = XDROP || (rt ? s_i : s_j) + MB <= (rt ? qlen : rlen) || (rt ? s_j : s_i) + MB <= (rt ? rlen : qlen);
+                if (TRACE) e = e && s_nb < nb_lim;
+                return e;
+            };
+            {
+                uint32_t qlen = qlen_r, rlen = rlen_r, nb_lim = 0;
+                if constexpr (TRACE) { const int4 b4 = *(const int4*)(lsc + MQ_LSC_PAIR + 4); qlen = (uint32_t)b4.x; rlen = (uint32_t)b4.y; nb_lim = (uint32_t)b4.z; }
+                leave = live && !eligible(si, sj, dir, nblocks, qlen, rlen, nb_lim);
+            }
+            static_assert(4u * MB + (SPM == 1 ? MB : 0u) <= BUFL, "the first step's stores stay inside the slot's buffer 0");
+            typedef __attribute__((address_space(1))) uint32_t* glb_u32_ptr;
+            typedef __attribute__((address_space(1))) vec_v4i* glb_v4i_ptr;
+            typedef int vec_v2i __attribute__((ext_vector_type(2)));
+            typedef __attribute__((address_space(1))) vec_v2i* glb_v2i_ptr;
+            glb_u32_ptr tw = (glb_u32_ptr)(uintptr_t)slot_mem + 8 * l;
+            int zw[2] = {0, 0}, tacc[8] = {0, 0, 0, 0, 0, 0, 0, 0};
+            bool commit = false;
+            auto store_words = [&]() {
+                if constexpr (TRACE) {
+#ifndef MQ_X_NOTRSTORE
+                    *(glb_v4i_ptr)tw = vec_v4i{tacc[0], tacc[1], tacc[2], tacc[3]}; *(glb_v4i_ptr)(tw + 4) = vec_v4i{tacc[4], tacc[5], tacc[6], tacc[7]};
+#else
+                    asm volatile("" :: "v"(tacc[0]), "v"(tacc[1]), "v"(tacc[2]), "v"(tacc[3]), "v"(tacc[4]), "v"(tacc[5]), "v"(tacc[6]), "v"(tacc[7]));
+#endif
+                    if constexpr (SPM == 1) *(glb_v2i_ptr)(tw - 8 * l + 128 + 2 * l) = vec_v2i{zw[0], zw[1]};
+                }
+            };
+            if (!__any(leave)) {
+            {
+                unsigned long long qa = qa_r, ra = ra_r;
+                if constexpr (TRACE) {
+                    const int4 a4 = *(const int4*)(lsc + MQ_LSC_PAIR);
+                    qa = (unsigned long long)bp.pool + ((unsigned long long)(uint32_t)a4.x | ((unsigned long long)(uint32_t)a4.y << 32));
+                    ra = (unsigned long long)bp.pool + ((unsigned long long)(uint32_t)a4.z | ((unsigned long long)(uint32_t)a4.w << 32));
+                }
+                const uint32_t* a = (const uint32_t*)((const uint8_t*)qa + (si + 8u * (uint32_t)l)); const uint32_t* b = (const uint32_t*)((const uint8_t*)ra + (sj + 8u * (uint32_t)l));
+                const uint32_t* cq = (const uint32_t*)((const uint8_t*)qa + si + (MB - STEP)); const uint32_t* cr = (const uint32_t*)((const uint8_t*)ra + sj + (MB - STEP));
+                pf_qv.x = a[0]; pf_qv.y = a[1]; pf_rv.x = b[0]; pf_rv.y = b[1];
+                pf_qc.x = cq[0]; pf_qc.y = cq[1]; pf_rc.x = cr[0]; pf_rc.y = cr[1];
+                asm volatile("" : "+v"(pf_qv.x), "+v"(pf_qv.y), "+v"(pf_rv.x), "+v"(pf_rv.y), "+v"(pf_qc.x), "+v"(pf_qc.y), "+v"(pf_rc.x), "+v"(pf_rc.y),
+                                  "+v"(mc.laneKG), "+v"(mc.lanem1KG), "+v"(mc.w0), "+v"(tw));
+            }
             do {
+                store_words();
                 const bool right = dir == DIR_RIGHT;
                 uint32_t lid;
                 asm volatile("v_mbcnt_lo_u32_b32 %0, -1, 0\n\tv_mbcnt_hi_u32_b32 %0, -1, %0" : "=v"(lid));
@@ -621,7 +665,6 @@
                 const __attribute__((address_space(4))) BatchParams* kargs = (const __attribute__((address_space(4))) BatchParams*)__builtin_amdgcn_kernarg_segment_ptr();
                 asm volatile("" : "+s"(kargs));
                 const glb_cu8_ptr pool_g = (glb_cu8_ptr)kargs->pool;
-                const bool pool64 = TRACE && (kargs->flags & (uint32_t)F_POOL64);
                 int4 cA = {0, 0, 0, 0}, cB = {0, 0, 0, 0}, cC = {0, 0, 0, 0};
                 if (TRACE) {
                     typedef const __attribute__((address_space(3))) lds_v4i* lds_cint4_ptr;
@@ -633,60 +676,42 @@
                 const uint32_t qo32 = (uint32_t)cA.x, ro32 = (uint32_t)cA.z;
                 const uint32_t qlen = TRACE ? (uint32_t)cB.x : qlen_r, rlen = TRACE ? (uint32_t)cB.y : rlen_r;
                 const uint32_t ri = right ? si : sj, rj = (right ? sj : si) + (MB - STEP);
-                const uint32_t lenV = right ? qlen : rlen, lenC = right ? rlen : qlen;
                 const bool q_out = si + MB > qlen, r_out = sj + MB > rlen;
-                bool elig = XDROP || ri + MB <= lenV || rj + STEP <= lenC;
                 const uint32_t trace_top = tt0 + nblocks * MQ_TW;
-                if (TRACE) elig = elig && nblocks < (uint32_t)cB.z;
-                leave = live && !elig;
-                const bool run = live && !leave;
                 const int off_n = off_max;
                 const int off_add = sat16(off - off_n);
                 const int corner = (prev_dir != dir && prev_dir != DIR_GROW) ? sat16(D_corner + off_add) : 0;
 #ifndef MQ_X_NOSTAGE
-                if (live) stage(lbuf_s, lsc_s, sel ^ 1u, si, sj, off_n, trace_top, nblocks, dir, off_add, corner);
+                stage(lbuf_s, lsc_s, sel ^ 1u, si, sj, off_n, trace_top, nblocks, dir, off_add, corner);
 #endif
                 asm volatile("" : "+v"(mc.laneKG), "+v"(mc.lanem1KG), "+v"(mc.w0));
-                uint2 vb, cbv;
+                uint2 vb = right ? pf_qv : pf_rv, cbv = {0, 0};
+                if constexpr (TRACE) cbv = right ? pf_rc : pf_qc;
+                asm volatile("" : "+v"(vb.x), "+v"(vb.y));
                 {
-                    const uint8_t* Vp = right ? qp : rp; const uint8_t* Cp = right ? rp : qp;
-                    vb = right ? pf_qv : pf_rv; cbv = right ? pf_rc : pf_qc;
-                    if (__any(run && !pf_ok)) {
-                        if (run && !pf_ok) {
-                            if constexpr (TRACE) {
-                                const unsigned long long vo = right ? ((unsigned long long)(uint32_t)cA.x | ((unsigned long long)(uint32_t)cA.y << 32)) : ((unsigned long long)(uint32_t)cA.z | ((unsigned long long)(uint32_t)cA.w << 32));
-                                const unsigned long long co = right ? ((unsigned long long)(uint32_t)cA.z | ((unsigned long long)(uint32_t)cA.w << 32)) : ((unsigned long long)(uint32_t)cA.x | ((unsigned long long)(uint32_t)cA.y << 32));
-                                const glb_cu32_ptr vp = (glb_cu32_ptr)(pool_g + (vo + (ri + l8))), cp = (glb_cu32_ptr)(pool_g + (co + rj));
-                                vb.x = vp[0]; vb.y = vp[1]; cbv.x = cp[0]; cbv.y = cp[1];
-                            } else {
-                            const uint32_t* vp = (const uint32_t*)(Vp + (ri + l8));
-                            vb.x = vp[0]; vb.y = vp[1];
-                            const uint32_t* cp = (const uint32_t*)(Cp + rj);
-                            cbv.x = cp[0]; cbv.y = cp[1];
-                            }
-                        }
-                    }
-                    asm volatile("" : "+v"(vb.x), "+v"(vb.y));
-                    if (!pool64) if (run) {
-                        if constexpr (TRACE) {
-                            const glb_cu32_ptr a = (glb_cu32_ptr)(pool_g + (unsigned long long)(qo32 + (si + l8))), b = (glb_cu32_ptr)(pool_g + (unsigned long long)(ro32 + (sj + l8)));
-                            const glb_cu32_ptr cq = (glb_cu32_ptr)(pool_g + (unsigned long long)(qo32 + si) + MB), cr = (glb_cu32_ptr)(pool_g + (unsigned long long)(ro32 + sj) + MB);
-                            pf_qv.x = a[0]; pf_qv.y = a[1]; pf_rv.x = b[0]; pf_rv.y = b[1];
-                            pf_qc.x = cq[0]; pf_qc.y = cq[1]; pf_rc.x = cr[0]; pf_rc.y = cr[1];
-                        } else {
+                    if constexpr (TRACE && P64) {
+                        const unsigned long long qo = (unsigned long long)(uint32_t)cA.x | ((unsigned long long)(uint32_t)cA.y << 32), ro = (unsigned long long)(uint32_t)cA.z | ((unsigned long long)(uint32_t)cA.w << 32);
+                        const glb_cu32_ptr a = (glb_cu32_ptr)(pool_g + (qo + (si + l8))), b = (glb_cu32_ptr)(pool_g + (ro + (sj + l8)));
+                        const glb_cu32_ptr cq = (glb_cu32_ptr)(pool_g + (qo + si) + MB), cr = (glb_cu32_ptr)(pool_g + (ro + sj) + MB);
+                        pf_qv.x = a[0]; pf_qv.y = a[1]; pf_rv.x = b[0]; pf_rv.y = b[1];
+                        pf_qc.x = cq[0]; pf_qc.y = cq[1]; pf_rc.x = cr[0]; pf_rc.y = cr[1];
+                    } else if constexpr (TRACE) {
+                        const glb_cu32_ptr a = (glb_cu32_ptr)(pool_g + (unsigned long long)(qo32 + (si + l8))), b = (glb_cu32_ptr)(pool_g + (unsigned long long)(ro32 + (sj + l8)));
+                        const glb_cu32_ptr cq = (glb_cu32_ptr)(pool_g + (unsigned long long)(qo32 + si) + MB), cr = (glb_cu32_ptr)(pool_g + (unsigned long long)(ro32 + sj) + MB);
+                        pf_qv.x = a[0]; pf_qv.y = a[1]; pf_rv.x = b[0]; pf_rv.y = b[1];
+                        pf_qc.x = cq[0]; pf_qc.y = cq[1]; pf_rc.x = cr[0]; pf_rc.y = cr[1];
+                    } else {
                         const uint32_t* a = (const uint32_t*)(qp + (si + l8)); const uint32_t* b = (const uint32_t*)(rp + (sj + l8));
                         const uint32_t* cq = (const uint32_t*)(qp + si + MB); const uint32_t* cr = (const uint32_t*)(rp + sj + MB);
                         pf_qv.x = a[0]; pf_qv.y = a[1]; pf_rv.x = b[0]; pf_rv.y = b[1];
+                        asm volatile("" : "+v"(pf_qc.x), "+v"(pf_qc.y), "+v"(pf_rc.x), "+v"(pf_rc.y) :: "memory");
+                        cbv = right ? pf_rc : pf_qc;
                         pf_qc.x = cq[0]; pf_qc.y = cq[1]; pf_rc.x = cr[0]; pf_rc.y = cr[1];
-                        }
-                        pf_ok = true;
                     }
                 }
-                uint32_t* tw = nullptr;
                 if (TRACE) {
-                    typedef __attribute__((address_space(1))) uint32_t* glb_u32_ptr;
-                    tw = (uint32_t*)(glb_u32_ptr)((unsigned long long)(uint32_t)cC.x | ((unsigned long long)(uint32_t)cC.y << 32)) + (trace_top + l8);
-                    if (run && l == 0) {
+                    tw = (glb_u32_ptr)((unsigned long long)(uint32_t)cC.x | ((unsigned long long)(uint32_t)cC.y << 32)) + (trace_top + l8);
+                    {
                         static_assert(sizeof(BlockRec) == 16, "a record as four words");
                         const uint32_t hw = right ? ((uint32_t)MB | ((uint32_t)STEP << 16)) : ((uint32_t)STEP | ((uint32_t)MB << 16));
                         typedef __attribute__((address_space(1))) vec_v4i* glb_rec_ptr;
@@ -695,11 +720,8 @@
                     }
                 }
                 MultiOut o;
-                int zw[2] = {0, 0};
-                multi_rect<KIND, TRACE, SPM, SL>(smem, fq, mc, l, A_d, A_c, P_d, P_r, vb, cbv.x, cbv.y, corner, off_add, tw, run, o, SPM ? splat(sat16(ZERO - off_n)) : 0,
+                multi_rect<KIND, TRACE, SPM, SL>(smem, fq, mc, l, A_d, A_c, P_d, P_r, vb, cbv.x, cbv.y, corner, off_add, tacc, o, (int)lid, SPM ? splat(sat16(ZERO - off_n)) : 0,
                                              SPM == 2 && right && ri == 0u && l == 0, zw);
-                if (TRACE && SPM == 1 && run) *(int2*)(tw - 8 * l + 128 + 2 * l) = int2{zw[0], zw[1]};
-
                 const int right_max = right ? o.act_max8 : o.pas_max8, down_max = right ? o.pas_max8 : o.act_max8;
                 const int new_off_max = off_n + o.mx - ZERO;
                 const bool improve = new_off_max > best_max;
@@ -707,8 +729,8 @@
                 bool stop = q_out && r_out;
                 if (XDROP) stop = stop || (!improve && new_off_max < best_max - x_drop && x_iter >= 1);
                 stop = stop || (!q_out && !r_out && 2 * MB <= max_size && new_y > MB / STEP - 1);
-                const bool commit = run && !stop;
-                leave = leave || (run && stop);
+                commit = live && !stop;
+                rolled = live && stop;
                 {
                     const bool imp = commit && improve;
                     if (keep_pre) sel ^= imp ? 1u : 0u;
@@ -731,9 +753,12 @@
 #ifdef BA_TIMING
                 n_quad++;
 #endif
+                leave = rolled || (live && !eligible(si, sj, dir, nblocks, qlen, rlen, (uint32_t)cB.z));
             } while (!__any(leave));
+            if (commit) store_words();
+            }
             const uint32_t trace_top = tt0 + nblocks * MQ_TW;
-            if (live && !leave) stage((uint32_t)(uintptr_t)(lbuf + l * 16), (uint32_t)(uintptr_t)lsc, sel ^ 1u, si, sj, 0, trace_top, nblocks, dir, 0, 0);
+            if (live && !rolled) stage((uint32_t)(uintptr_t)(lbuf + l * 16), (uint32_t)(uintptr_t)lsc, sel ^ 1u, si, sj, 0, trace_top, nblocks, dir, 0, 0);
             lds_sync();
             if (live) {
 #pragma unroll
@@ -748,10 +773,12 @@
             lds_sync();
             if (live && l == 0) {
                 int* rc = (int*)(slot_mem + 2 * BUFA);
-                const uint32_t nsteps = (uint32_t)mq_load((const char*)(rc + MR_NSTEPS)) + ((si + sj) - (uint32_t)mq_load((const char*)(rc + MR_SI)) - (uint32_t)mq_load((const char*)(rc + MR_SJ))) / (uint32_t)STEP;
+                const uint32_t taken = ((si + sj) - (uint32_t)mq_load((const char*)(rc + MR_SI)) - (uint32_t)mq_load((const char*)(rc + MR_SJ))) / (uint32_t)STEP;
+                const uint32_t nsteps = (uint32_t)mq_load((const char*)(rc + MR_NSTEPS)) + taken;
                 rc[MR_SI] = (int)si; rc[MR_SJ] = (int)sj; rc[MR_DIR] = dir; rc[MR_PREV_DIR] = prev_dir; rc[MR_OFF] = off; rc[MR_OFF_MAX] = off_max; rc[MR_BEST_MAX] = best_max;
                 rc[MR_Y_DROP] = (int)y_drop; rc[MR_X_ITER] = x_iter; rc[MR_D_CORNER] = D_corner; rc[MR_NSTEPS] = (int)nsteps; rc[MR_TRACE_TOP] = (int)trace_top;
                 rc[MR_NBLOCKS] = (int)nblocks; rc[MR_SEL] = (int)sel;
+                if (bp.flags & F_COUNT_STEPS) atomicAdd(bp.prof + (P64 ? 49 : 48), (unsigned long long)taken);
             }
             const unsigned long long lm = __ballot(leave && l == 0);
             pend_m = 0;
@@ -795,6 +822,15 @@
     }
 }
 
+template <int PMAX, int KIND, bool TRACE, bool XDROP, int SPM = 0, int MBP = 128, int WPW = WAVES_PER_WG, int EU = MQ_WAVES_EU>
+__global__ void __launch_bounds__(WPW * 64, (PMAX >= 16 ? 2 : EU)) k_multi(const BatchParams bp) {
+    multi_body<PMAX, KIND, TRACE, XDROP, SPM, MBP, WPW, EU, false>(bp);
+}
+template <int PMAX, int KIND, bool XDROP, int SPM = 0, int MBP = 128, int WPW = WAVES_PER_WG, int EU = MQ_WAVES_EU>
+__global__ void __launch_bounds__(WPW * 64, (PMAX >= 16 ? 2 : EU)) k_multi_p64(const BatchParams bp) {
+    multi_body<PMAX, KIND, true, XDROP, SPM, MBP, WPW, EU, true>(bp);
+}
+
 #undef don_final
 #undef don_offers
 }
diff --git a/block_aligner_amd/csrc/ba_params.h b/block_aligner_amd/csrc/ba_params.h
--- a/block_aligner_amd/csrc/ba_params.h
+++ b/block_aligner_amd/csrc/ba_params.h
@@ -11,6 +11,7 @@
 enum : uint32_t {
     F_TRACE = 1u << 0, F_XDROP = 1u << 1, F_LOCAL = 1u << 2, F_FQS = 1u << 3, F_FQE = 1u << 4, F_CIGAR_EQ = 1u << 5,
     F_POOL64 = 1u << 15,
+    F_COUNT_STEPS = 1u << 16,
     F_PAD_NEG = 1u << 14
 };
 enum : uint32_t { ST_OK = 0, ST_TRACE_OVERFLOW = 1, ST_BLOCKS_OVERFLOW = 2, ST_CIGAR_OVERFLOW = 4, ST_TRACEBACK_LOST = 8, ST_WATCHDOG = 16, ST_SLOT_TIMEOUT = 32, ST_MODE = 64,
```

New measurement: 2697 (median of 6 runs). +1.2%, better.
